# SymbolicML/DynamicExpressions.jl

Measured on AMD Instinct MI355X. Metric: node-evals/sec, higher is better.
Workload: dtype f32

## Files before the change

### dynamicexpressions.jl_amd/api.py

```python
from __future__ import annotations

import ctypes as C
import math
import os
from dataclasses import dataclass
from typing import Optional, Sequence, Tuple, Union

import numpy as np

from .node import Node, TAPE_DTYPE, count_constant_nodes, flatten_graph, flatten_population, max_feature, preserve_sharing
from .operators import OperatorEnum

_HERE = os.path.dirname(os.path.abspath(__file__))
LIB_PATH = os.environ.get("DE_HIP_LIB") or os.path.join(_HERE, "csrc", "libde_hip.so")

DE_F32, DE_F64, DE_F16, DE_CF32, DE_CF64 = 0, 1, 2, 3, 4
COMPLEX_DTYPES = (np.dtype(np.complex64), np.dtype(np.complex128))
GRAD_VARIABLE, GRAD_CONSTANT, GRAD_BOTH = 0, 1, 2
ABI_VERSION = 3
OPT_EARLY_EXIT, OPT_FUSE_DEG1, OPT_FUSE_DEG2, OPT_BUMPER_CHECKS, OPT_TURBO, OPT_FULL_EVAL, OPT_FORWARD_GRAD, OPT_REVERSE_GRAD = 1, 2, 4, 8, 16, 32, 64, 128

EXPORTS = [
    "de_abi_version", "de_opcode_table_version", "de_opcode_by_name", "de_opcode_name",
    "de_opcode_degree", "de_status_string", "de_ctx_create", "de_ctx_destroy", "de_ctx_set_stream",
    "de_ctx_synchronize", "de_ctx_declare_dataset", "de_ctx_stream", "de_last_error", "de_program_create", "de_program_create_cse",
    "de_program_set_consts", "de_program_update", "de_program_destroy", "de_program_n_trees", "de_program_n_nodes",
    "de_program_n_grad", "de_program_dump", "de_program_verify", "de_program_stream_hash", "de_host_pool_selftest", "de_lower_tape", "de_lower_tape_stage", "de_lower_tape_complex", "de_lower_tape_stage_complex", "de_lower_tape_grad", "de_eval", "de_eval_grad", "de_eval_diff", "de_eval_loss", "de_eval_loss_grad", "de_eval_loss_grad_by_class",
    "de_loss_spec_check", "de_eval_loss_ex", "de_eval_fit_stats", "de_eval_loss_gn", "de_gn_max_rows", "de_eval_loss_grad_ex", "de_eval_loss_grad_by_class_ex",
    "de_eval_pullback_dX", "de_eval_tree_array", "de_eval_plan", "de_prio_tiles_wanted", "de_program_last_live_trees", "de_dist_unique_id", "de_dist_init", "de_dist_destroy", "de_dist_shard_size", "de_dist_world_size",
    "de_dist_broadcast", "de_dist_gather_flags", "de_dist_last_error", "de_ctx_last_kernel_ms", "de_ctx_last_kernel_name",
    "de_ctx_device", "de_ctx_timing_ring", "de_ctx_timing_read", "de_dist_reorder_selftest", "de_eval_sum_certificate",
    "de_dist_set_timeout", "de_ctx_trim", "de_program_set_consts_device", "de_program_get_consts", "de_program_consts_device_path",
    "de_lower_tape_assured", "de_lower_tape_assured_parts", "de_gn_lm_step", "de_fit_consts_lm", "de_lm_solve_host",
    "de_gn_spec_check", "de_eval_loss_gn_ex", "de_fit_consts_lm_ex", "de_eval_fit_stats_grad",
    "de_gn_wide_max_rows", "de_eval_loss_gn_wide", "de_lm_solve_host_wide", "de_gn_lm_step_wide", "de_fit_consts_lm_wide",
    "de_lm_project_host", "de_fit_stats_lm_step", "de_fit_consts_lm_scaled",
    "de_eval_fit_stats_grad_wide", "de_lm_project_host_wide", "de_fit_stats_lm_step_wide", "de_fit_consts_lm_scaled_wide",
    "de_bfgs_max_rows", "de_bfgs_direction_host", "de_bfgs_update_host", "de_fit_consts_bfgs",
    "de_tape_params_to_consts", "de_eval_tree_params", "de_eval_loss_tree_params", "de_eval_loss_grad_tree_params",
    "de_tree_params_accumulate_host",
    "de_fit_tree_params_bfgs", "de_tree_params_pack_host", "de_tree_params_unpack_host",
]


class DeviceError(RuntimeError):
    """The HIP library/GPU is unavailable or a de_* call failed.  Never swallowed."""


class UncertifiedFlag(DeviceError):
    """EvalContext(strict_flags=True): the device's element-wise validity flag of this tree is not PROVABLY the reference's
    `isfinite(sum(x))` flag (a finite array whose sum may overflow): the caller keeps the CPU path for it."""


class ParamArgs(C.Structure):
    _fields_ = [("params", C.c_void_p), ("ld_params", C.c_int64), ("n_classes", C.c_int64),
                ("classes", C.c_void_p), ("classes_is_i64", C.c_int32), ("class_base", C.c_int32)]


class LossSpec(C.Structure):
    _fields_ = [("kind", C.c_int32), ("reserved", C.c_int32), ("param", C.c_double)]


class LmOpts(C.Structure):
    _fields_ = [("iters", C.c_int32), ("reserved", C.c_int32), ("lam0", C.c_double), ("up", C.c_double), ("down", C.c_double),
                ("lam_min", C.c_double)]


class TreeParams(C.Structure):
    _fields_ = [("params", C.c_void_p), ("ld_params", C.c_int64), ("n_classes", C.c_int64), ("n_params", C.c_int32),
                ("reserved", C.c_int32), ("class_starts", C.c_void_p), ("slot_param", C.c_void_p)]


class BfgsOpts(C.Structure):
    _fields_ = [("iters", C.c_int32), ("reserved", C.c_int32), ("step0", C.c_double), ("shrink", C.c_double), ("c1", C.c_double),
                ("curv", C.c_double)]


LOSS_KINDS = {"L2": 0, "L1": 1, "pullback": 2, "huber": 16, "logcosh": 17, "l1_eps": 18, "l2_eps": 19, "quantile": 20, "lp": 21,
              "logit_dist": 22, "logit_margin": 23, "l1_hinge": 24}


def loss_spec(loss: str, loss_param: float = 0.0, with_gradient: bool = True) -> LossSpec:
    if loss == "pullback" and not with_gradient:
        raise KeyError(loss)
    spec = LossSpec(LOSS_KINDS[loss], 0, float(loss_param))
    if library().de_loss_spec_check(C.byref(spec), int(with_gradient)) != 0:
        raise ValueError(f"loss {loss!r}: parameter {loss_param!r} is not finite or outside the kind's range (include/de_hip.h de_loss_kind_t)")
    return spec


def gn_loss_spec(loss: str, loss_param: float = 0.0, e_floor: float = 1e-4) -> LossSpec:
    spec = LossSpec(LOSS_KINDS[loss], 0, float(loss_param))
    rc = library().de_gn_spec_check(C.byref(spec), float(e_floor))
    if rc == 7:
# ... 375 lines not shown
    if lib.de_abi_version() != ABI_VERSION:
        raise DeviceError(f"{LIB_PATH} has ABI version {lib.de_abi_version()}, this module was written for {ABI_VERSION}: rebuild (csrc/build.sh)")
    lib.de_opcode_table_version.restype = C.c_int
    lib.de_opcode_by_name.argtypes = [C.c_char_p, C.c_int]
    lib.de_opcode_name.restype = C.c_char_p
    lib.de_opcode_name.argtypes = [C.c_int]
    lib.de_opcode_degree.argtypes = [C.c_int]
    lib.de_status_string.restype = C.c_char_p
    lib.de_status_string.argtypes = [C.c_int]
    lib.de_ctx_create.argtypes = [C.c_int, vp, C.POINTER(vp)]
    lib.de_ctx_destroy.argtypes = [vp]
    lib.de_ctx_set_stream.argtypes = [vp, vp]
    lib.de_ctx_synchronize.argtypes = [vp]
    lib.de_ctx_declare_dataset.argtypes = [vp, C.c_int, vp, i64, i64, i32]
    lib.de_ctx_stream.restype = vp
    lib.de_ctx_stream.argtypes = [vp]
    lib.de_last_error.restype = C.c_char_p
    lib.de_last_error.argtypes = [vp]
    lib.de_program_create.argtypes = [vp, C.c_int, vp, vp, i64, vp, vp, i32, i32, u32, C.POINTER(vp)]
    lib.de_program_create_cse.argtypes = [vp, C.c_int, vp, vp, vp, vp, i64, vp, vp, i32, i32, u32, C.POINTER(vp)]
    lib.de_program_set_consts.argtypes = [vp, vp]
    lib.de_program_set_consts_device.argtypes = [vp, vp]
    lib.de_program_get_consts.argtypes = [vp, vp]
    lib.de_program_consts_device_path.argtypes = [vp]
    lib.de_program_update.argtypes = [vp, vp, i64, vp, vp, vp, vp, vp, vp]
    lib.de_program_destroy.argtypes = [vp]
    lib.de_program_n_trees.restype = i64
    lib.de_program_n_trees.argtypes = [vp]
    lib.de_program_n_nodes.restype = i64
    lib.de_program_n_nodes.argtypes = [vp]
    lib.de_program_n_grad.restype = i64
    lib.de_program_n_grad.argtypes = [vp, i64, C.c_int]
    lib.de_program_verify.argtypes = [vp]
    lib.de_host_pool_selftest.restype = C.c_int64
    lib.de_host_pool_selftest.argtypes = [C.c_int64, C.POINTER(C.c_int32)]
    lib.de_program_stream_hash.restype = C.c_uint64
    lib.de_program_stream_hash.argtypes = [vp]
    lib.de_program_dump.restype = i64
    lib.de_program_dump.argtypes = [vp, i64, vp, i64, C.c_int]
    lib.de_lower_tape.restype = i64
    lib.de_lower_tape.argtypes = [C.c_int, vp, i64, vp, i64, i32, i32, u32, vp, i64, vp]
    lib.de_lower_tape_stage.restype = i64
    lib.de_lower_tape_stage.argtypes = [C.c_int, vp, i64, vp, i64, i32, i32, u32, C.c_int, vp, i64]
    for fn in (lib.de_lower_tape_complex, lib.de_lower_tape_stage_complex):
        fn.restype = i64
    lib.de_lower_tape_complex.argtypes = lib.de_lower_tape.argtypes
    lib.de_lower_tape_stage_complex.argtypes = lib.de_lower_tape_stage.argtypes
    if hasattr(lib, "de_lower_tape_assured"):
        lib.de_lower_tape_assured.restype = i64
        lib.de_lower_tape_assured.argtypes = [vp, i64, vp, i64, i32, u32, C.c_double, vp, i64]
    if hasattr(lib, "de_lower_tape_assured_parts"):
        lib.de_lower_tape_assured_parts.restype = i64
        lib.de_lower_tape_assured_parts.argtypes = [vp, i64, vp, i64, i32, u32, C.c_double, u32, vp, i64]
    lib.de_lower_tape_grad.restype = i64
    lib.de_lower_tape_grad.argtypes = [C.c_int, vp, i64, vp, i64, i32, i32, u32, C.c_int, C.c_int, vp, i64, vp]
    lib.de_eval.argtypes = [vp, vp, vp, i64, i64, C.POINTER(ParamArgs), vp, i64, vp]
    lib.de_eval_loss.argtypes = [vp, vp, vp, i64, i64, C.POINTER(ParamArgs), vp, vp, C.c_int32, vp, vp]
    lib.de_eval_loss_grad.argtypes = [vp, vp, vp, i64, i64, C.POINTER(ParamArgs), C.c_int, vp, vp, C.c_int32, vp, vp, vp, vp]
    lib.de_eval_loss_grad_by_class.argtypes = [vp, vp, vp, i64, i64, C.POINTER(ParamArgs), C.c_int, vp, vp, C.c_int32, vp, vp, vp, vp, vp, vp]
    lib.de_loss_spec_check.argtypes = [C.POINTER(LossSpec), C.c_int]
    lib.de_eval_loss_ex.argtypes = [vp, vp, vp, i64, i64, C.POINTER(ParamArgs), vp, vp, C.POINTER(LossSpec), vp, vp]
    lib.de_eval_fit_stats.argtypes = [vp, vp, vp, i64, i64, C.POINTER(ParamArgs), vp, vp, vp, vp, vp]
    lib.de_eval_loss_gn.argtypes = [vp, vp, vp, i64, i64, C.POINTER(ParamArgs), C.c_int, vp, vp, vp, vp, vp, vp, vp, vp]
    lib.de_gn_max_rows.argtypes = []
    if hasattr(lib, "de_fit_consts_lm"):
        lib.de_gn_lm_step.argtypes = [vp, C.c_int, i64, vp, vp, vp, vp, vp, vp, vp, vp]
        lib.de_fit_consts_lm.argtypes = [vp, vp, vp, i64, i64, C.POINTER(ParamArgs), vp, vp, C.POINTER(LmOpts), vp, vp, vp, vp]
        lib.de_lm_solve_host.argtypes = [C.c_int, vp, vp, C.c_double, vp]
    if hasattr(lib, "de_gn_spec_check"):
        lib.de_gn_spec_check.argtypes = [C.POINTER(LossSpec), C.c_double]
        lib.de_eval_loss_gn_ex.argtypes = [vp, vp, vp, i64, i64, C.POINTER(ParamArgs), C.c_int, vp, vp, C.POINTER(LossSpec), C.c_double,
                                           vp, vp, vp, vp, vp, vp]
        lib.de_fit_consts_lm_ex.argtypes = [vp, vp, vp, i64, i64, C.POINTER(ParamArgs), vp, vp, C.POINTER(LossSpec), C.c_double,
                                            C.POINTER(LmOpts), vp, vp, vp, vp]
    if hasattr(lib, "de_eval_fit_stats_grad"):
        lib.de_eval_fit_stats_grad.argtypes = [vp, vp, vp, i64, i64, C.POINTER(ParamArgs), C.c_int, vp, vp, vp, vp, vp, vp, vp, vp, vp]
    if hasattr(lib, "de_eval_loss_gn_wide"):
        lib.de_gn_wide_max_rows.argtypes = []
        lib.de_eval_loss_gn_wide.argtypes = lib.de_eval_loss_gn_ex.argtypes
        lib.de_lm_solve_host_wide.argtypes = lib.de_lm_solve_host.argtypes
        lib.de_gn_lm_step_wide.argtypes = lib.de_gn_lm_step.argtypes
        lib.de_fit_consts_lm_wide.argtypes = lib.de_fit_consts_lm_ex.argtypes
    if hasattr(lib, "de_fit_consts_lm_scaled"):
        lib.de_lm_project_host.argtypes = [C.c_int, vp, vp, vp, vp, vp, vp, vp]
        lib.de_fit_stats_lm_step.argtypes = [vp, C.c_int, i64, vp, vp, vp, vp, vp, vp, vp, vp, vp, vp, vp]
        lib.de_fit_consts_lm_scaled.argtypes = [vp, vp, vp, i64, i64, C.POINTER(ParamArgs), vp, vp, C.POINTER(LmOpts), vp, vp, vp, vp, vp, vp]
    if hasattr(lib, "de_fit_consts_lm_scaled_wide"):
        lib.de_eval_fit_stats_grad_wide.argtypes = lib.de_eval_fit_stats_grad.argtypes
        lib.de_lm_project_host_wide.argtypes = lib.de_lm_project_host.argtypes
        lib.de_fit_stats_lm_step_wide.argtypes = lib.de_fit_stats_lm_step.argtypes
        lib.de_fit_consts_lm_scaled_wide.argtypes = lib.de_fit_consts_lm_scaled.argtypes
    if hasattr(lib, "de_fit_consts_bfgs"):
        lib.de_bfgs_max_rows.argtypes = []
        lib.de_bfgs_direction_host.argtypes = [C.c_int, vp, vp, vp, vp, C.c_double, vp, vp]
        lib.de_bfgs_update_host.argtypes = [C.c_int, vp, vp, vp, vp, C.c_double]
        lib.de_fit_consts_bfgs.argtypes = [vp, vp, vp, i64, i64, C.POINTER(ParamArgs), vp, vp, C.POINTER(LossSpec), C.POINTER(BfgsOpts),
                                           vp, vp, vp, vp]
    if hasattr(lib, "de_eval_tree_params"):
        lib.de_tape_params_to_consts.restype = i64
        lib.de_tape_params_to_consts.argtypes = [vp, i64, i32, vp, vp, i64]
        lib.de_eval_tree_params.argtypes = [vp, vp, vp, i64, i64, C.POINTER(TreeParams), vp, i64, vp]
        lib.de_eval_loss_tree_params.argtypes = [vp, vp, vp, i64, i64, C.POINTER(TreeParams), vp, vp, C.POINTER(LossSpec), vp, vp]
        lib.de_eval_loss_grad_tree_params.argtypes = [vp, vp, vp, i64, i64, C.POINTER(TreeParams), vp, vp, C.POINTER(LossSpec), vp, vp, vp, vp, vp]
        lib.de_tree_params_accumulate_host.argtypes = [C.c_int, i32, vp, i32, i64, vp, vp, vp, vp, vp, vp, vp, vp]
    if hasattr(lib, "de_fit_tree_params_bfgs"):
        lib.de_fit_tree_params_bfgs.argtypes = [vp, vp, vp, i64, i64, C.POINTER(TreeParams), vp, vp, C.POINTER(LossSpec), C.POINTER(BfgsOpts),
# ... 195 lines not shown
        if not (X.stride(0) == 1 and (N <= 1 or X.stride(1) >= F)) and X.numel() > 0:
            X = X.t().contiguous().t()
        ld = X.stride(1) if N > 1 else max(F, 1)
        return X.data_ptr(), F, N, ld, X, True
    X = np.asarray(X)
    if X.ndim == 1:
        X = X.reshape(-1, 1)
    Xf = np.asfortranarray(X, dtype=dtype)
    F, N = Xf.shape
    return Xf.ctypes.data, F, N, max(F, 1), Xf, False


def lower_tape(tape, consts, n_features: int, n_params: int = 0, options: int = 7, dtype=np.float32):
    lib = library()
    dtype = np.dtype(dtype)
    tape = np.ascontiguousarray(tape)
    consts = np.ascontiguousarray(consts, dtype=dtype)
    meta = np.zeros(4, dtype=np.int32)
    cp = consts.ctypes.data if consts.size else None
    lower = lib.de_lower_tape_complex if dtype in COMPLEX_DTYPES else lib.de_lower_tape
    n = lower(_dtype_code(dtype), tape.ctypes.data, len(tape), cp, consts.size, n_features,
              n_params, options, None, 0, meta.ctypes.data)
    if n < 0:
        code = int(-n)
        name = lib.de_status_string(code).decode()
        if code == 3:
            from .operators import UnsupportedOperatorError
            raise UnsupportedOperatorError(name)
        raise ValueError(name)
    w = np.zeros(max(int(n), 1), dtype=np.uint32)
    lower(_dtype_code(dtype), tape.ctypes.data, len(tape), cp, consts.size, n_features,
          n_params, options, w.ctypes.data, w.size, meta.ctypes.data)
    return w[:int(n)].reshape(-1, 4), dict(n_slots=int(meta[0]), host_ok_eval=bool(meta[1]),
                                           host_ok_grad=bool(meta[2]), uses_params=bool(meta[3]))


def lower_tape_stage(tape, consts, n_features: int, stage: int, n_params: int = 0, options: int = 7,
                     dtype=np.float32) -> np.ndarray:
    lib = library()
    dtype = np.dtype(dtype)
    tape = np.ascontiguousarray(tape)
    consts = np.ascontiguousarray(consts, dtype=dtype)
    cp = consts.ctypes.data if consts.size else None
    args = (_dtype_code(dtype), tape.ctypes.data, len(tape), cp, consts.size, n_features, n_params, options, stage)
    stage_fn = lib.de_lower_tape_stage_complex if dtype in COMPLEX_DTYPES else lib.de_lower_tape_stage
    n = stage_fn(*args, None, 0)
    if n < 0:
        raise ValueError(lib.de_status_string(int(-n)).decode())
    w = np.zeros(max(int(n), 1), dtype=np.uint32)
    stage_fn(*args, w.ctypes.data, w.size)
    return w[:int(n)].reshape(-1, 4)


def lower_tape_assured(tape, consts, n_features: int, xmax: float = 64.0, options: int = 7, parts: Optional[int] = None) -> np.ndarray:
    lib = library()
    tape = np.ascontiguousarray(tape)
    consts = np.ascontiguousarray(consts, dtype=np.float32)
    cp = consts.ctypes.data if consts.size else None
    args = (tape.ctypes.data, len(tape), cp, consts.size, n_features, options, float(xmax))
    fn = lib.de_lower_tape_assured
    if parts is not None:
        fn, args = lib.de_lower_tape_assured_parts, args + (int(parts),)
    n = fn(*args, None, 0)
    if n < 0:
        raise ValueError(lib.de_status_string(int(-n)).decode())
    w = np.zeros(max(int(n), 1), dtype=np.float64)
    fn(*args, w.ctypes.data, w.size)
    return w[:int(n)].reshape(-1, 6)


def lower_tape_grad(tape, consts, n_features: int, mode: int, form: int, n_params: int = 0, options: int = 7, dtype=np.float32):
    lib = library()
    dtype = np.dtype(dtype)
    tape = np.ascontiguousarray(tape)
    consts = np.ascontiguousarray(consts, dtype=dtype)
    cp = consts.ctypes.data if consts.size else None
    meta = np.zeros(8, dtype=np.int32)
    args = (_dtype_code(dtype), tape.ctypes.data, len(tape), cp, consts.size, n_features, n_params, options, mode, form)
    n = lib.de_lower_tape_grad(*args, None, 0, meta.ctypes.data)
    if n < 0:
        raise ValueError(lib.de_status_string(int(-n)).decode())
    w = np.zeros(max(int(n), 1), dtype=np.uint32)
    lib.de_lower_tape_grad(*args, w.ctypes.data, w.size, meta.ctypes.data)
    return w[:int(n)].reshape(-1, 4), meta


def check_update_ids(indices, n_new: int, n_trees: int) -> np.ndarray:
    ids = np.asarray(list(indices) if not isinstance(indices, np.ndarray) else indices)
    if ids.ndim != 1:
        raise ValueError("update: indices must be one-dimensional")
    if len(ids) != n_new:
        raise ValueError(f"update: {len(ids)} indices for {n_new} trees")
    if len(ids) == 0:
        return np.zeros(0, dtype=np.int64)
    if ids.dtype.kind not in "iu":
        raise ValueError(f"update: indices must be integers, got {ids.dtype}")
    ids = np.ascontiguousarray(ids, dtype=np.int64)
    if ids.min() < 0 or ids.max() >= n_trees:
        raise ValueError(f"update: tree index outside [0, {n_trees})")
    if len(np.unique(ids)) != len(ids):
        raise ValueError("update: a tree index appears twice")
    return ids


class Population:

    def __init__(self, trees: Sequence[Node], operators: OperatorEnum, dtype=np.float32,
                 n_features: Optional[int] = None, n_params: int = 0,
                 eval_context: Optional[EvalContext] = None, ctx: Optional[Context] = None):
        self.ctx = ctx or default_context()
        self.dtype = np.dtype(dtype)
        self.operators = operators
        self.eval_context = eval_context or EvalContext()
        self.n_trees = len(trees)
# ... 138 lines not shown
        return library().de_program_consts_device_path(self._h) == 1

    def verify(self) -> None:
        self.ctx.check(library().de_program_verify(self._h))

    def stream_hash(self) -> int:
        return int(library().de_program_stream_hash(self._h))

    def _combine_rows(self, t: int, g, mode: int):
        if self._occ is None or self._occ[t] is None or mode == GRAD_VARIABLE:
            return g
        o = self._occ[t]
        lead = g.shape[0] - len(o)
        nu = int(o.max()) + 1
        if _is_torch(g):
            import torch
            out = torch.zeros((lead + nu,) + tuple(g.shape[1:]), dtype=g.dtype, device=g.device)
            out[:lead] = g[:lead]
            out.index_add_(0, torch.as_tensor(o + lead, device=g.device), g[lead:])
            return out
        out = np.zeros((lead + nu,) + g.shape[1:], dtype=g.dtype)
        out[:lead] = g[:lead]
        np.add.at(out, o + lead, g[lead:])
        return out

    def plan(self, N: int) -> dict:
        pl = np.zeros(3, dtype=np.int32)
        self.ctx.check(library().de_eval_plan(self._h, N, pl.ctypes.data))
        return dict(tile=int(pl[0]), n_chunks=int(pl[1]), trees_per_chunk=int(pl[2]))

    def last_live_trees(self) -> int:
        n = C.c_int64(-1)
        self.ctx.check(library().de_program_last_live_trees(self._h, C.byref(n)))
        return int(n.value)

    def n_grad(self, tree: int, mode: int) -> int:
        return int(library().de_program_n_grad(self._h, tree, mode))

    def _n_grad_all(self, mode: int) -> np.ndarray:
        cache = self.__dict__.setdefault("_ng_cache", {})
        if mode not in cache:
            lib = library()
            cache[mode] = np.array([lib.de_program_n_grad(self._h, t, mode) for t in range(self.n_trees)], dtype=np.int64)
        return cache[mode]

    def dump(self, tree: int) -> np.ndarray:
        lib = library()
        n = lib.de_program_dump(self._h, tree, None, 0, 0)
        w = np.zeros(max(int(n), 1), dtype=np.uint32)
        got = lib.de_program_dump(self._h, tree, w.ctypes.data, w.size, 0)
        return w[:int(got)].reshape(-1, 4)

    def meta(self, tree: int) -> dict:
        w = np.zeros(7, dtype=np.uint32)
        library().de_program_dump(self._h, tree, w.ctypes.data, 7, 1)
        return dict(n_slots=int(w[0]), host_ok_eval=bool(w[1]), host_ok_grad=bool(w[2]), uses_params=bool(w[3]), waves=int(w[4]),
                    assured=bool(w[5]), assured_valid=bool(w[6]))

    def dump_stage(self, tree: int, which: int) -> np.ndarray:
        lib = library()
        n = lib.de_program_dump(self._h, tree, None, 0, which)
        w = np.zeros(max(int(n), 1), dtype=np.uint32)
        got = lib.de_program_dump(self._h, tree, w.ctypes.data, w.size, which)
        return w[:int(got)].reshape(-1, 4)

    def _param_args(self, params, classes, class_base, N, keep):
        if self.n_params == 0 and params is None:
            return None
        if params is None or classes is None:
            raise ValueError("Incorrect call. You must pass the `classes::Vector` argument when calling `eval_tree_array`.")
        pa = ParamArgs()
        if _is_torch(params):
            import torch
            params = params.to(_torch_dtype(self.dtype))
            if params.stride(0) != 1 and params.numel() > 0:
                params = params.t().contiguous().t()
            P, ncls = params.shape
            pa.params, pa.ld_params = params.data_ptr(), (params.stride(1) if ncls > 1 else max(P, 1))
        else:
            params = np.asfortranarray(params, dtype=self.dtype)
            P, ncls = params.shape
            pa.params, pa.ld_params = params.ctypes.data, max(P, 1)
        if P != self.n_params:
            raise ValueError("parameter matrix has the wrong number of rows")
        if _is_torch(classes):
            import torch
            if classes.dtype not in (torch.int32, torch.int64):
                classes = classes.to(torch.int64)
            classes = classes.contiguous()
            n_c = classes.numel()
            key = (classes.data_ptr(), n_c, classes._version, ncls, class_base)
            if n_c and key not in self._classes_checked:
                mn, mx = int(classes.min().item()), int(classes.max().item())
                if mn < class_base or mx - class_base >= ncls:
                    raise ValueError(f"class ids must lie in [{class_base}, {class_base + ncls}): got [{mn}, {mx}] "
                                     "(maximum(classes) <= size(parameters, 2))")
                if len(self._classes_checked) > 64:
                    self._classes_checked.clear()
                self._classes_checked.add(key)
            pa.classes, pa.classes_is_i64 = classes.data_ptr(), int(classes.dtype == torch.int64)
        else:
            classes = np.ascontiguousarray(classes)
            if classes.dtype not in (np.int32, np.int64):
                classes = classes.astype(np.int64)
            n_c = classes.size
            if n_c:
                mn, mx = int(classes.min()), int(classes.max())
                if mn < class_base or mx - class_base >= ncls:
                    raise ValueError(f"class ids must lie in [{class_base}, {class_base + ncls}): got [{mn}, {mx}] "
                                     "(maximum(classes) <= size(parameters, 2))")
# ... 1367 lines not shown
```

### dynamicexpressions.jl_amd/csrc/de_api_eval.cpp

```cpp
#include "de_api_internal.h"

extern "C" {
int stage_in(de_ctx *c, DevBuf &buf, const void *user, size_t bytes, Staged *s) {
    s->dev = const_cast<void *>(user);
    s->staged = false;
    if (!user || bytes == 0 || is_device_ptr(user)) return DE_OK;
    HIP_TRY(c, buf.reserve(bytes));
    HIP_TRY(c, hipMemcpyAsync(buf.p, user, bytes, hipMemcpyHostToDevice, c->stream));
    s->dev = buf.p;
    s->staged = true;
    return DE_OK;
}
int stage_out(de_ctx *c, DevBuf &buf, void *user, size_t bytes, Staged *s) {
    s->dev = user;
    s->staged = false;
    if (!user || bytes == 0 || is_device_ptr(user)) return DE_OK;
    HIP_TRY(c, buf.reserve(bytes));
    s->dev = buf.p;
    s->staged = true;
    return DE_OK;
}

int check_param_args(de_ctx *c, const de_program *p, const de_param_args_t *pa, int64_t N) {
    if (!p->uses_params) return DE_OK;
// ... 236 lines not shown
    if (ok_dev) {
        sOk.dev = ok;
    } else {
        HIP_TRY(c, c->sOk.reserve((size_t)p->n_trees));
        sOk.dev = c->sOk.p;
        sOk.staged = true;
    }
    if (!p->d_ok_eval) HIP_TRY(c, hipMemcpyAsync(sOk.dev, p->host_ok_eval.data(), (size_t)p->n_trees, hipMemcpyHostToDevice, c->stream));
    if (p->uses_params) {
        rc = stage_in(c, c->sParams, pa->params, (size_t)pa->ld_params * (size_t)pa->n_classes * es, &sPar);
        if (rc) return rc;
        rc = stage_in(c, c->sClasses, pa->classes, (size_t)N * (pa->classes_is_i64 ? 8 : 4), &sCls);
        if (rc) return rc;
    }
    EvalArgs a;
    std::memset(&a, 0, sizeof a);
    a.code = p->d_code;
    a.code_off = p->d_code_off;
    a.n_trees = (int32_t)p->n_trees;
    a.n_slots = p->n_slots + (p->prows ? p->n_params : 0);
    a.prow_base = p->prows ? p->n_features + p->n_slots : 0;
    a.n_prows = p->prows ? p->n_params : 0;
    a.uses_params = p->uses_params;
    a.X = sX.dev;
    a.N = N;
    a.ldX = ldX;
    a.F = p->n_features;
    a.out = sOut.dev;
    a.ld_out = ld_out;
    a.ok = static_cast<uint8_t *>(sOk.dev);
    a.ok_init = p->d_ok_eval;
    if (p->uses_params) {
        a.params = sPar.dev;
        a.ld_params = pa->ld_params;
        a.n_classes = pa->n_classes;
        a.classes = sCls.dev;
        a.classes_is_i64 = pa->classes_is_i64;
        a.class_base = pa->class_base;
    }
    a.early_exit = (p->options & DE_OPT_EARLY_EXIT) != 0;
    a.skip_flagged = a.early_exit && !(p->options & DE_OPT_FULL_EVAL) && tree_skip_enabled();
    a.turbo = (p->options & DE_OPT_TURBO) != 0;
    a.threaded = p->threaded && !direct;
    a.direct = direct;
    a.loss = lr ? &la : nullptr;
    HIP_TRY(c, c->sPrio.reserve((size_t)3 * DE_PRIO_MAX_F * sizeof(unsigned long long)));
    a.prio_keys = c->sPrio.p;
    a.prio_keys_ready = !half && !cplx && !sX.staged && dataset_keys(c, p->dtype, X, N, ldX, p->n_features, &a.prio_keys);
    a.compact_code = p->d_compact_code;
    a.compact_ints = p->d_compact_ints;
    a.waves = p->waves;
    a.wave_slots = p->n_slots;
    a.var_stride = p->var_stride;
    a.assured = p->assured && p->assured_valid && p->var_stride != 0;
    a.assured_xmax = (float)p->assured_xmax;
    if (cr) {
        a.code = p->d_cert_code;
        a.code_off = p->d_cert_off;
        a.threaded = false;
        a.cert_max = c->sCert.p;
        a.out = nullptr;
        a.prio_keys = nullptr;
        a.compact_code = nullptr;
        a.compact_ints = nullptr;
    }
    if (!c->nested) HIP_TRY(c, time_begin(c));
    a.compacted = &p->last_compacted;
    p->last_compacted = false;
    if (half || cplx) {
        a.threaded = false;
        a.prio_keys = nullptr;
        a.compact_code = nullptr;
        a.compact_ints = nullptr;
    }
    if (half) HIP_TRY(c, launch_eval_f16(a, c->stream, &c->last_kernel));
    else if (cplx) HIP_TRY(c, launch_eval_complex(p->io, a, p->d_ctab, c->stream, &c->last_kernel));
    else HIP_TRY(c, launch_eval(p->dtype, a, c->stream, &c->last_kernel));
    if (!c->nested) HIP_TRY(c, time_end(c));
    if (sLoss.staged) HIP_TRY(c, hipMemcpyAsync(lr->loss, sLoss.dev, (size_t)p->n_trees * es, hipMemcpyDeviceToHost, c->stream));
    if (sStats.staged) HIP_TRY(c, hipMemcpyAsync(lr->stats, sStats.dev, (size_t)p->n_trees * 3 * sizeof(double), hipMemcpyDeviceToHost, c->stream));
    if (sYstats.staged) HIP_TRY(c, hipMemcpyAsync(lr->ystats, sYstats.dev, 3 * sizeof(double), hipMemcpyDeviceToHost, c->stream));
    if (sOut.staged) {
        if (ld_out == N)
            HIP_TRY(c, hipMemcpyAsync(out, sOut.dev, (size_t)p->n_trees * (size_t)N * es, hipMemcpyDeviceToHost, c->stream));
        else
            for (int64_t t = 0; t < p->n_trees; t++)
                HIP_TRY(c, hipMemcpyAsync(static_cast<char *>(out) + (size_t)t * (size_t)ld_out * es,
                                          static_cast<char *>(sOut.dev) + (size_t)t * (size_t)ld_out * es,
                                          (size_t)N * es, hipMemcpyDeviceToHost, c->stream));
    }
    if (sOk.staged) HIP_TRY(c, hipMemcpyAsync(ok, sOk.dev, (size_t)p->n_trees, hipMemcpyDeviceToHost, c->stream));
    if (cr) {
        std::vector<unsigned char> mx((size_t)p->n_trees * ces);
        std::vector<uint8_t> okh((size_t)p->n_trees);
        HIP_TRY(c, hipMemcpyAsync(mx.data(), c->sCert.p, mx.size(), hipMemcpyDeviceToHost, c->stream));
        HIP_TRY(c, hipMemcpyAsync(okh.data(), sOk.dev, okh.size(), hipMemcpyDeviceToHost, c->stream));
        HIP_TRY(c, hipStreamSynchronize(c->stream));
        const double top = half ? 65504.0 : p->dtype == DE_F32 ? (double)std::numeric_limits<float>::max() : std::numeric_limits<double>::max();
        double margin = 1.001;
        if (half) {
            const double d = 1024.0 + std::ceil(std::log2(std::max(1.0, (double)N / 1024.0))) + 8.0;
            margin = std::exp(d * std::log1p(std::ldexp(1.0, -11)));
        }
        for (int64_t t = 0; t < p->n_trees; t++) {
            double m = p->dtype == DE_F32 ? (double)reinterpret_cast<float *>(mx.data())[t] : reinterpret_cast<double *>(mx.data())[t];
            m = std::max(m, p->cert_cmax[(size_t)t]);
            if (cr->max_abs) cr->max_abs[t] = m;
            cr->certified[t] = (!okh[(size_t)t] || m * (double)N * margin < top || !(m == m)) ? 1 : 0;
// ... 41 lines not shown
```

### dynamicexpressions.jl_amd/csrc/de_api_internal.h

```cpp
#ifndef DE_API_INTERNAL_H
#define DE_API_INTERNAL_H
#include <hip/hip_runtime.h>
#include <pthread.h>

#include <chrono>
#include <cmath>
#include <cstdarg>
#include <cstdio>
#include <cstring>
#include <condition_variable>
#include <functional>
#include <map>
#include <mutex>
#include <memory>
#include <new>
#include <string>
#include <algorithm>
#include <array>
#include <atomic>
#include <thread>
#include <vector>

#include "../../include/de_hip.h"
#include "de_kernels.h"
// ... 71 lines not shown
    int dtype = DE_F32;
    int io = DE_F32;
    std::vector<double> consts_im, ctab;
    void *d_ctab = nullptr;
    uint32_t options = 0;
    int32_t n_features = 0, n_params = 0;
    int64_t n_trees = 0, n_nodes = 0;
    int n_slots = 0;
    bool prows = false;
    bool uses_params = false;
    std::vector<Instr> code;
    std::vector<int32_t> code_off;
    std::vector<int64_t> const_off;
    std::vector<int32_t> const_instr;
    std::vector<uint8_t> const_checks;
    std::vector<int32_t> n_consts_tree;
    bool cse_generic = false;
    std::vector<uint8_t> host_ok_eval;
    std::vector<uint8_t> host_ok_grad;
    std::vector<double> consts;
    bool folded = false;
    std::vector<Instr> fcode;
    std::vector<int32_t> fcode_off;
    std::vector<int32_t> fconst_instr;
    struct Fold { int32_t tree, instr; bool tested_always; };
    std::vector<Fold> folds;
    std::vector<int64_t> aux_const_src;
    de_program *aux = nullptr;
    std::vector<uint8_t> fold_ok;
    std::vector<uint8_t> fold_host;
    std::vector<int32_t> kfold;
    std::vector<int64_t> kf_csrc;
    char *d_kf = nullptr;
    size_t kf_o_noff = 0, kf_o_coff = 0, kf_o_cvals = 0, kf_o_out = 0, kf_o_ok = 0, kf_bytes = 0;
    std::vector<de_tape_node_t> fold_nodes;
    std::vector<int64_t> fold_noff, fold_coff;
    std::vector<int32_t> aux_fold;
    std::vector<int64_t> aux_csrc;
    std::vector<BoundInstr> bcode;
    std::vector<BoundInstr> tcode;
    std::vector<BoundInstr> fbcode;
    std::vector<int32_t> tcode_off;
    std::vector<BoundInstr> ccode;
    std::vector<int32_t> ccode_off;
    int waves = 1;
    int waves_choice = 0;
    int64_t var_stride = 0;
    std::vector<BoundInstr> ccode_w;
    bool assured = false, assured_valid = false;
    int assured_cfg = 0;
    double assured_xmax = 64.0;
    uint32_t assured_parts = 0;
    std::vector<uint32_t> aids;
    uint64_t end_handler = 0;
    uint64_t endv_handler[TOPX_ENDV_COUNT] = {0};
    bool threaded = false;
    bool direct = false;
    uint64_t handler_base = 0;
    std::vector<int32_t> bcode_off;
    BoundInstr *d_code = nullptr;
    int32_t *d_code_off = nullptr;
    bool eval_arena = false;
    BoundInstr *d_compact_code = nullptr;
    int32_t *d_compact_ints = nullptr;
    bool last_compacted = false;
    BoundInstr *d_cert_code = nullptr;
    int32_t *d_cert_off = nullptr;
    size_t cert_cap = 0;
    uint64_t consts_gen = 0;
    uint64_t cert_gen = ~0ull;
    std::vector<double> cert_cmax;
    BoundInstr *d_gcode = nullptr;
    int32_t *d_gcode_off = nullptr;
    std::vector<BoundInstr> gbcode;
    std::vector<int32_t> gbcode_off;
    bool gcode_stale = true;
    std::vector<BoundInstr> gtcode;
    std::vector<int32_t> gtcode_off;
    BoundInstr *d_gtcode = nullptr;
    int32_t *d_gtcode_off = nullptr;
    int32_t *d_gt_ids = nullptr;
    uint8_t *d_ok_eval = nullptr;
    uint8_t *d_ok_grad = nullptr;
    int32_t *d_ng = nullptr;
    int64_t *d_goff = nullptr;
    int tab_mode = -1;
    int64_t tab_N = -1;
    bool tab_ok_stale = true;
    std::vector<int32_t> bsite, tsite, gbsite, gtsite_of_gb;
    struct EvalSite { int32_t src, b, t, c; };
    struct GradSite { int32_t src, gb, gt, rt; };
    std::vector<EvalSite> eval_sites;
    std::vector<GradSite> grad_sites;
    uint64_t site_gen = 1, lists_gen = 0;
    std::vector<BoundInstr> rtcode;
    std::vector<int32_t> rtcode_off, rtcode_mid, rtsite_of_gb;
    BoundInstr *d_rtcode = nullptr;
    int32_t *d_rtcode_off = nullptr, *d_rtcode_mid = nullptr, *d_rt_ids = nullptr;
    int rt_mode = -1, rt_stage_cols = 0, rt_n_groups = 0;
    GradArgs::RevGroup rt_groups[8];
    bool rt_valid = false;
    uint64_t rt_handler_base = 0;
    uint32_t rt_param_off = 0;
    int gt_mode = -1;
    bool gt_valid = false, gt_wide = false;
    bool gt_share = false;
// ... 128 lines not shown
```

### dynamicexpressions.jl_amd/csrc/de_api_program.cpp

```cpp
#include "de_api_internal.h"
#include "de_const_patch.h"

template <typename T>
static bool host_fold_eval(const de_tape_node_t *nd, int64_t n, const double *consts, const int64_t *csrc, T *value, bool half = false) {
    T stack_small[32];
    std::vector<T> stack_big;
    T *st = stack_small;
    if (n > 32) { stack_big.resize((size_t)n); st = stack_big.data(); }
    int sp = 0;
    bool ok = true;
    for (int64_t i = 0; i < n; i++) {
        T v;
        if (nd[i].degree == 0) v = (T)consts[csrc[nd[i].arg]];
        else {
            const T b = st[--sp], a = st[--sp];
            switch (nd[i].op) {
            case DE_B_ADD: v = a + b; break;
            case DE_B_SUB: v = a - b; break;
            case DE_B_MUL: v = a * b; break;
            default: v = a / b; break;
            }
            if (half) v = (T)(_Float16)v;
        }
        ok = ok && std::isfinite(v);
// ... 81 lines not shown
    const std::vector<Instr> &src = p->folded ? p->fcode : p->code;
    const std::vector<int32_t> &off = p->folded ? p->fcode_off : p->code_off;
    const int nf = p->n_features;
    const de_program *old = ru && ru->old && same_binding(p, ru->old) ? ru->old : nullptr;
    build_stream_by_trees<BoundInstr>(p->n_trees, &p->bcode, &p->bcode_off, [&](int64_t t, std::vector<BoundInstr> *out) {
        if (old && ru->src[(size_t)t] >= 0) {
            const size_t s = (size_t)ru->src[(size_t)t];
            out->insert(out->end(), old->bcode.begin() + old->bcode_off[s], old->bcode.begin() + old->bcode_off[s + 1]);
            return;
        }
        const int32_t i0 = off[(size_t)t], i1 = off[(size_t)t + 1];
        bind_tree(src.data() + i0, (size_t)(i1 - i0), ee, nf, out, prb);
    });
    match_const_sites(src, off, p->bcode, p->bcode_off, p->n_trees, [](const BoundInstr &b) { return bop_is_const_source(b.bop); }, &p->bsite);
    p->tsite.clear();
    p->site_gen++;
}

static void make_chained(de_program *p);
static int choose_waves(const de_program *p) {
    if (TBLK != 64 || (p->uses_params && !p->prows)) return 1;
    if (const char *e = getenv("DE_EVAL_WAVES")) { const int v = atoi(e); return (v == 2 || v == 4 || v == 8) ? v : 1; }
    const size_t rb = trow_bytes(p->dtype), lds_cu = 160u << 10, shared = (size_t)p->n_features + (p->prows ? (size_t)p->n_params : 0);
    auto resident = [&](int W) -> size_t {
        const size_t lds = (shared + (size_t)W * (size_t)p->n_slots) * rb + (size_t)W * 256;
        const size_t by_regs = W >= 4 ? 7 / ((size_t)W / 4) : 28 / (size_t)W;
        return lds > 150u * 1024 ? 0 : std::min<size_t>(lds_cu / lds, by_regs) * (size_t)W;
    };
    int best = 1;
    size_t have = resident(1);
    for (int W : {2, 4, 8}) {
        const size_t w = resident(W);
        if (have >= 20) break;
        if (w * 2 < have * 3) {
            if (W == 2 && have < 12) continue;
            break;
        }
        best = W;
        have = w;
    }
    return best;
}
static void make_assured(de_program *p, const uint64_t *table);
static double assured_xmax_env() {
    const char *ax = getenv("DE_ASSURED_XMAX");
    const double xm = ax ? (double)(float)atof(ax) : 64.0;
    return (xm >= 0x1p-40 && xm <= 0x1p100) ? xm : 64.0;
}
static uint32_t assured_parts_env() {
    const char *ap = getenv("DE_ASSURED_PARTS");
    const int v = ap && *ap ? atoi(ap) : (int)ASSURED_PARTS_SHIPPED;
    return (uint32_t)v & ASSURED_PARTS_ALL;
}
static int make_threaded(de_ctx *c, de_program *p, const Reuse *ru = nullptr) {
    p->threaded = false;
    p->waves = 1;
    p->var_stride = 0;
    p->ccode_w.clear();
    p->assured = p->assured_valid = false;
    p->aids.clear();
    if (p->assured_cfg == 0) {
        if (ru && ru->old && ru->old->assured_cfg != 0) {
            p->assured_cfg = ru->old->assured_cfg;
            p->assured_xmax = ru->old->assured_xmax;
            p->assured_parts = ru->old->assured_parts;
        } else {
            const char *as = getenv("DE_ASSURED");
            p->assured_parts = assured_parts_env();
            p->assured_cfg = ((as && *as == '0') || p->assured_parts == 0) ? -1 : 1;
            p->assured_xmax = assured_xmax_env();
        }
    }
    dbg_lap(nullptr);
    p->direct = (size_t)eval_rows(p) * FLAT_ROW_BYTES > 150 * 1024;
    if (p->io == DE_F16) return DE_OK;
    if (is_complex_io(p->io)) {
        p->direct = (size_t)eval_rows(p) * complex_row_bytes(p->io) > 64 * 1024;
        return DE_OK;
    }
    if ((p->direct && ((size_t)eval_rows(p) + 3 * (size_t)p->n_slots) * trow_bytes(p->dtype) + 4 * 256 > 150 * 1024) || !eval_uses_threaded()) return DE_OK;
    if (eval_rows(p) > 4000) return DE_OK;
    uint64_t table[TOPX_TABLE];
    hipError_t st = eval_handler_table(p->dtype, (p->options & DE_OPT_TURBO) != 0, table);
    if (st != hipSuccess) return fail(c, DE_ERR_HIP, "handler table: %s", hipGetErrorString(st));
    dbg_lap("handler table");
    uint64_t base = table[0];
    for (int i = 0; i < (int)TOPX_TABLE; i++) base = std::min<uint64_t>(base, table[i]);
    for (int i = 0; i < (int)TOPX_TABLE; i++) {
        if (table[i] - base > 0xFFFFFFFFull) return DE_OK;
        if (p->dtype != DE_F32 && (table[i] >> 32) != (table[0] >> 32)) return DE_OK;
    }
    const bool hot_unary = !getenv("DE_NO_CONST_UNARY_HOT");
    const uint32_t row_bytes = (uint32_t)trow_bytes(p->dtype);
    const char *nf = getenv("DE_NO_FUSE");
    const bool fuse = !(nf && *nf == '1');
    if (p->waves_choice == 0) p->waves_choice = choose_waves(p);
    const int W = fuse ? p->waves_choice : 1;
    const int wave_prows = p->prows ? p->n_params : 0;
    const FuseRows rows0{(uint32_t)p->n_features, (uint32_t)(p->n_features + p->n_slots), 0, W > 1 ? wave_prows + (W - 1) * p->n_slots : 0};
    const de_program *old = ru && ru->old && ru->old->threaded && ru->old->waves_choice == p->waves_choice && same_binding(p, ru->old) ? ru->old : nullptr;
    build_stream_by_trees<BoundInstr>(p->n_trees, &p->fbcode, &p->tcode_off, [&](int64_t t, std::vector<BoundInstr> *out) {
        if (old && ru->src[(size_t)t] >= 0) {
            const size_t s = (size_t)ru->src[(size_t)t];
            out->insert(out->end(), old->fbcode.begin() + old->tcode_off[s], old->fbcode.begin() + old->tcode_off[s + 1]);
            return;
        }
        const int32_t b0 = p->bcode_off[(size_t)t], b1 = p->bcode_off[(size_t)t + 1];
        if (fuse) fuse_tree(p->bcode.data() + b0, (size_t)(b1 - b0), out, W > 1 && p->n_slots > 0 ? &rows0 : nullptr);
        else out->insert(out->end(), p->bcode.begin() + b0, p->bcode.begin() + b1);
    });
    dbg_lap("fuse_tree");
    p->tcode.resize(p->fbcode.size());
    auto threaded_words = [p, &table, base, hot_unary, row_bytes](const BoundInstr &b) {
        BoundInstr t = b;
        t.bop = (uint32_t)(table[b.bop] - base);
        if (hot_unary && (b.bop == BOP_GEN_ROW || b.bop == BOP_GEN_ACC)) {
            const int k = gun_index((int)(b.arg >> 24), DE_U_COS, DE_U_EXP, DE_U_SIN, DE_U_NEG, DE_U_SQUARE, DE_U_CUBE, DE_U_ABS, DE_U_LOG, DE_U_SAFE_LOG,
                                    DE_U_SQRT, DE_U_SAFE_SQRT, DE_U_TANH, DE_U_RELU);
            if (k >= 3) t.bop = (uint32_t)(table[TOPX_UN_BASE + (uint32_t)(k - 3) * 2 + (b.bop == BOP_GEN_ACC ? 1 : 0)] - base);
        }
        if (hot_unary && (b.bop == BOP_GEN_ROW || b.bop == BOP_GEN_CONST) && ((b.arg >> 24) == (uint32_t)DE_B_MAX || (b.arg >> 24) == (uint32_t)DE_B_MIN))
            t.bop = (uint32_t)(table[TOPX_BIN_BASE + ((b.arg >> 24) == (uint32_t)DE_B_MAX ? 0u : 2u) + (b.bop == BOP_GEN_CONST ? 1u : 0u)] - base);
        if (b.bop < BOP_COUNT && bop_is_const_source(b.bop)) {
// ... 100 lines not shown
        r.bop = la;
        if (f32) r.arg = lo;
        else { r.lo = lo; r.hi = hi; }
    };
    auto name_next = [&](BoundInstr &r, uint64_t handler) {
        if (f32) { r.lo = (uint32_t)handler; r.hi = (uint32_t)(handler >> 32); }
        else r.arg = (uint32_t)handler;
    };
    auto ev_of = [&](int64_t t) -> int {
        const int32_t i0 = p->tcode_off[(size_t)t], i1 = p->tcode_off[(size_t)t + 1];
        return i1 - i0 >= 2 ? topx_endv_of(p->fbcode[(size_t)i1 - 1].bop) : -1;
    };
    auto handler_of = [&](int32_t i, int32_t i1, int ev) -> uint64_t {
        return (i == i1 - 1 && ev >= 0) ? p->endv_handler[ev] : p->handler_base + p->tcode[(size_t)i].bop;
    };
    parallel_tree_ranges(p->n_trees, [&](int, int64_t tb, int64_t te) {
        for (int64_t t = tb; t < te; t++) {
            const int32_t i0 = p->tcode_off[(size_t)t], i1 = p->tcode_off[(size_t)t + 1];
            const size_t h = (size_t)i0 + (size_t)t + 1;
            p->ccode_off[(size_t)t] = (int32_t)h;
            const int ev = ev_of(t);
            for (int32_t i = i0; i < i1; i++) {
                const BoundInstr &s = p->tcode[(size_t)i];
                put(p->ccode[h + (size_t)(i - i0)], s.arg, s.lo, s.hi);
                if (i > i0) name_next(p->ccode[h + (size_t)(i - i0) - 1], handler_of(i, i1, ev));
            }
            put(p->ccode[h + (size_t)(i1 - i0)], (uint32_t)t, 0u, 0u);
            if (i1 > i0) name_next(p->ccode[h + (size_t)(i1 - i0) - 1], p->end_handler);
        }
    });
    for (int64_t t = 0; t < p->n_trees; t++) {
        const int32_t i0 = p->tcode_off[(size_t)t], i1 = p->tcode_off[(size_t)t + 1];
        const size_t h = (size_t)p->ccode_off[(size_t)t];
        const int ev = ev_of(t);
        if (i1 > i0) {
            const uint64_t first = handler_of(i0, i1, ev);
            name_next(p->ccode[h - 1], first);
            if (t > 0 && ev_of(t - 1) >= 0) name_next(p->ccode[h - 2], first);
        } else name_next(p->ccode[h - 1], p->end_handler);
        put(p->ccode[h - 1], t == 0 ? 0u : (uint32_t)(t - 1), (uint32_t)(i1 - i0) | (ev >= 0 ? DE_HDR_FUSED_END : 0u), 0u);
    }
    if (p->n_trees > 0) name_next(p->ccode.back(), p->end_handler);
    p->ccode_off[(size_t)p->n_trees] = (int32_t)p->ccode.size();
}
static inline void patch_chained_imm(de_program *p, int32_t c, uint32_t lo, uint32_t hi) {
    if (p->dtype == DE_F32) p->ccode[(size_t)c].arg = lo;
    else { p->ccode[(size_t)c].lo = lo; p->ccode[(size_t)c].hi = hi; }
    for (size_t w = 0; w * p->ccode.size() < p->ccode_w.size(); w++) {
        BoundInstr &r = p->ccode_w[w * p->ccode.size() + (size_t)c];
        if (p->dtype == DE_F32) r.arg = lo;
        else { r.lo = lo; r.hi = hi; }
    }
}
static void assured_link_trees(de_program *p, const uint64_t *table, int64_t tb, int64_t te, bool touched_only = false) {
    BoundInstr *cw = p->ccode_w.data();
    std::vector<AssuredInstr> info;
    auto name_next = [](BoundInstr &r, uint64_t handler) { r.lo = (uint32_t)handler; r.hi = (uint32_t)(handler >> 32); };
    auto ev_of = [&](int64_t t) -> int {
        const int32_t i0 = p->tcode_off[(size_t)t], i1 = p->tcode_off[(size_t)t + 1];
        return i1 - i0 >= 2 ? topx_endv_of(p->fbcode[(size_t)i1 - 1].bop) : -1;
    };
    for (int64_t t = tb; t < te; t++) {
        const int32_t i0 = p->tcode_off[(size_t)t], i1 = p->tcode_off[(size_t)t + 1];
        if (i1 <= i0) continue;
        if (touched_only && p->const_off[(size_t)t + 1] == p->const_off[(size_t)t]) continue;
        info.resize((size_t)(i1 - i0));
        assure_tree(p->fbcode.data() + i0, (size_t)(i1 - i0), p->n_features, p->assured_xmax, info.data(), p->assured_parts);
        const size_t h = (size_t)p->ccode_off[(size_t)t];
        const int ev = ev_of(t);
        for (int32_t i = i0; i < i1; i++) {
            const uint32_t id = info[(size_t)(i - i0)].id;
            p->aids[(size_t)i] = id;
            const uint64_t handler = (i == i1 - 1 && ev >= 0) ? (topx_enda_of(id) >= 0 && id != p->fbcode[(size_t)i].bop ? table[TOPX_ENDA_BASE + (uint32_t)topx_enda_of(id)] : p->endv_handler[ev])
                                     : id == p->fbcode[(size_t)i].bop ? p->handler_base + p->tcode[(size_t)i].bop : table[id];
            if (i > i0) name_next(cw[h + (size_t)(i - i0) - 1], handler);
            else {
                name_next(cw[h - 1], handler);
                if (t > 0 && ev_of(t - 1) >= 0) name_next(cw[h - 2], handler);
            }
        }
    }
}
static void make_assured(de_program *p, const uint64_t *table) {
    p->ccode_w = p->ccode;
    p->aids.assign(p->fbcode.size(), 0u);
    parallel_tree_ranges(p->n_trees, [&](int, int64_t tb, int64_t te) { assured_link_trees(p, table, tb, te); });
    p->var_stride = (int64_t)(p->bcode.size() + (size_t)p->n_trees + 2);
    p->assured = p->assured_valid = true;
}
static hipError_t upload_wave_variants(de_program *p) {
    for (size_t w = 0; p->var_stride && w * p->ccode.size() < p->ccode_w.size(); w++) {
        const hipError_t st = hipMemcpy(p->d_code + (w + 1) * (size_t)p->var_stride, p->ccode_w.data() + w * p->ccode.size(),
                                        p->ccode.size() * sizeof(BoundInstr), hipMemcpyHostToDevice);
        if (st != hipSuccess) return st;
    }
    return hipSuccess;
}

static void recompute_host_ok(de_program *p) {
    const bool ee = (p->options & DE_OPT_EARLY_EXIT) != 0;
    parallel_for_trees(p->n_trees, [&](int64_t t) {
        bool ok_eval = true, ok_grad = true;
        for (int64_t k = p->const_off[t]; k < p->const_off[t + 1]; k++) {
            const bool fin = finite_in(p->dtype, p->consts[k]) && (p->consts_im.empty() || finite_in(p->dtype, p->consts_im[k]));
            ok_grad = ok_grad && fin;
            const uint8_t ch = p->const_checks[k];
            if (!fin && ((ch & CONST_CHECK_ALWAYS) || (ee && (ch & CONST_CHECK_EE)))) ok_eval = false;
        }
        p->host_ok_eval[t] = ok_eval;
        p->host_ok_grad[t] = ok_grad;
    }, 1024);
    for (size_t j = 0; j < p->folds.size() && j < p->fold_ok.size(); j++)
        if (!p->fold_ok[j] && (p->folds[j].tested_always || ee)) p->host_ok_eval[(size_t)p->folds[j].tree] = 0;
}

static int create_impl(de_ctx_t *ctx, int dtype, const de_tape_node_t *nodes, const int64_t *node_offsets,
                       int64_t n_trees, const void *consts, const int64_t *const_offsets, int32_t n_features,
                       int32_t n_params, uint32_t options, bool allow_fold, de_program_t **out_program,
                       const de_tape_node_t *cse_nodes = nullptr, const int64_t *cse_offsets = nullptr, const Reuse *reuse = nullptr,
                       bool keep_input = true);

static int upload_ok_eval(de_ctx *c, de_program *p) {
    p->tab_ok_stale = true;
    if (p->n_trees == 0) return DE_OK;
    if (!p->d_ok_eval) HIP_TRY(c, hipMalloc(reinterpret_cast<void **>(&p->d_ok_eval), (size_t)std::max<int64_t>(p->n_trees, 1)));
    HIP_TRY(c, hipStreamSynchronize(c->stream));
    HIP_TRY(c, hipMemcpy(p->d_ok_eval, p->host_ok_eval.data(), (size_t)p->n_trees, hipMemcpyHostToDevice));
    return DE_OK;
}

static int refresh_folds(de_ctx *c, de_program *p, bool aux_current = false) {
    if (!p->folded || p->folds.empty()) return DE_OK;
    const size_t es = p->dtype == DE_F32 ? 4 : 8;
    const size_t ies = dtype_bytes(p->io);
    const size_t nf = p->folds.size();
    p->fold_ok.assign(nf, 0);
    parallel_for_trees((int64_t)nf, [&](int64_t j) {
        if (p->fold_host[(size_t)j] != 1) return;
        const de_tape_node_t *nd = p->fold_nodes.data() + p->fold_noff[(size_t)j];
// ... 564 lines not shown
                        std::vector<int32_t> oaux(o->folds.size(), -1);
                        for (size_t a = 0; a < o->aux_fold.size(); a++) oaux[(size_t)o->aux_fold[a]] = (int32_t)a;
                        aru.old = o->aux;
                        aru.src.assign(p->aux_fold.size(), -1);
                        for (size_t a = 0; a < p->aux_fold.size(); a++) {
                            const size_t j = (size_t)p->aux_fold[a];
                            const int64_t t = p->folds[j].tree;
                            if (!reuse->reuse(t)) continue;
                            const size_t s = (size_t)reuse->src[(size_t)t];
                            aru.src[a] = oaux[(size_t)(reuse->fold0[s] + ((int64_t)j - fold0[(size_t)t]))];
                        }
                        aru.fold0.assign((size_t)o->aux->n_trees + 1, 0);
                        for (const de_program::Fold &f : o->aux->folds) aru.fold0[(size_t)f.tree + 1]++;
                        for (size_t q = 0; q < (size_t)o->aux->n_trees; q++) aru.fold0[q + 1] += aru.fold0[q];
                    }
                    int rc = create_impl(ctx, io, xnodes.data(), xnoff.data(), (int64_t)p->aux_fold.size(), ac.data(),
                                         xcoff.data(), n_features, 0, options, false, &p->aux, nullptr, nullptr, aru.old ? &aru : nullptr,
                                         false);
                    if (rc != DE_OK) return rc;
                    lap("aux program (create)");
                }
                int rc = refresh_folds(ctx, p.get(), true);
                if (rc != DE_OK) return rc;
                lap("folds (evaluate: host + kernel + aux)");
            } else if (any_cse) {
                p->folded = true;
            } else {
                p->fcode.clear();
                p->fcode_off.clear();
            }
        }
        if (!allow_fold) parallel_for_trees(n_trees, [&](int64_t t) { Lowered done; std::swap(done, low[(size_t)t]); });
        lap("release lowerings");
        if (cplx) fill_ctab_consts(p.get());
        recompute_host_ok(p.get());
        rebind(p.get(), reuse);
        lap("bind");
    } catch (const std::bad_alloc &) {
        return fail(ctx, DE_ERR_HIP, "out of host memory");
    }
    HIP_TRY(ctx, hipSetDevice(ctx->device));
    {
        int rc = DE_OK;
        try { rc = make_threaded(ctx, p.get(), reuse); } catch (const std::bad_alloc &) { rc = fail(ctx, DE_ERR_HIP, "out of host memory"); }
        if (rc != DE_OK) return rc;
    }
    lap("threaded + chained records");
    if (cplx) {
        const int rc = upload_ctab(ctx, p.get());
        if (rc != DE_OK) return rc;
    }
    const size_t cbytes = (p->bcode.size() + (size_t)p->n_trees + 2) * sizeof(BoundInstr);
    {
        const size_t nvar = p->threaded && p->var_stride ? (p->assured ? 2 : (size_t)p->waves) : 1;
        if (nvar > 1 && (size_t)p->var_stride * sizeof(BoundInstr) != cbytes) return fail(ctx, DE_ERR_HIP, "wave-group stream variants: stride and arena disagree");
        const size_t abytes = p->threaded ? 2 * nvar * cbytes : cbytes;
        auto al = [](size_t x) { return (x + 255) & ~(size_t)255; };
        const size_t off_bytes = p->bcode_off.size() * sizeof(int32_t);
        const size_t ints_bytes = p->threaded ? ((size_t)2 * (size_t)p->n_trees + 5) * sizeof(int32_t) : 0;
        const size_t o_off = al(abytes), o_ints = o_off + al(off_bytes), o_ok = o_ints + al(ints_bytes);
        const size_t total = o_ok + al((size_t)std::max<int64_t>(p->n_trees, 1));
        const hipError_t ast = prog_malloc(ctx, reinterpret_cast<void **>(&p->d_code), total);
        if (ast != hipSuccess) return fail(ctx, DE_ERR_HIP, "hipMalloc failed: %s", hipGetErrorString(ast));
        if (!in_one_window(p->d_code, abytes)) return fail(ctx, DE_ERR_HIP, "instruction stream straddles a 4 GiB boundary");
        char *base = reinterpret_cast<char *>(p->d_code);
        p->eval_arena = true;
        p->d_code_off = reinterpret_cast<int32_t *>(base + o_off);
        p->d_ok_eval = reinterpret_cast<uint8_t *>(base + o_ok);
        if (p->threaded) {
            p->d_compact_code = p->d_code + nvar * cbytes / sizeof(BoundInstr);
            p->d_compact_ints = reinterpret_cast<int32_t *>(base + o_ints);
        }
        lap("hipMalloc (arena)");
        const std::vector<BoundInstr> &stream = p->threaded ? p->ccode : p->bcode;
        const std::vector<int32_t> &offs = p->threaded ? p->ccode_off : p->bcode_off;
        hipError_t st = hipSuccess;
        if (total <= (size_t)(128u << 10)) {
            std::vector<unsigned char> img(total, 0);
            if (!stream.empty()) std::memcpy(img.data(), stream.data(), stream.size() * sizeof(BoundInstr));
            for (size_t w = 1; w < nvar; w++)
                std::memcpy(img.data() + w * cbytes, p->ccode_w.data() + (w - 1) * p->ccode.size(), p->ccode.size() * sizeof(BoundInstr));
            std::memcpy(img.data() + o_off, offs.data(), off_bytes);
            if (p->n_trees > 0) std::memcpy(img.data() + o_ok, p->host_ok_eval.data(), (size_t)p->n_trees);
            st = hipMemcpy(base, img.data(), total, hipMemcpyHostToDevice);
        } else {
            st = hipMemset(p->d_code, 0, nvar * cbytes);
            if (st == hipSuccess && !stream.empty()) st = hipMemcpy(p->d_code, stream.data(), stream.size() * sizeof(BoundInstr), hipMemcpyHostToDevice);
            if (st == hipSuccess) st = upload_wave_variants(p.get());
            if (st == hipSuccess) st = hipMemcpy(p->d_code_off, offs.data(), off_bytes, hipMemcpyHostToDevice);
            if (st == hipSuccess && p->n_trees > 0) st = hipMemcpy(p->d_ok_eval, p->host_ok_eval.data(), (size_t)p->n_trees, hipMemcpyHostToDevice);
        }
        if (st != hipSuccess) {
            prog_free(ctx, p->d_code);
            p->d_code = nullptr;
            return fail(ctx, DE_ERR_HIP, "program upload failed: %s", hipGetErrorString(st));
        }
    }
    lap("memset + upload (stream, offsets, flags)");
    if (getenv("DE_VERIFY") && *getenv("DE_VERIFY") == '1') {
        const int rc = de_program_verify(p.get());
        if (rc != DE_OK) return rc;
    }
    *out_program = p.release();
    return DE_OK;
}

static void refresh_site_lists(de_program *p) {
// ... 66 lines not shown
    const auto t3 = now();
    if (cplx) return upload_ctab(ctx, p);
    const char *nopatch = getenv("DE_NO_CONST_PATCH");
    if (!(nopatch && *nopatch == '1') && p->threaded && !p->tsite.empty() && !p->bsite.empty()) {
        const std::vector<Instr> &src = p->folded ? p->fcode : p->code;
        const bool gpatch = p->d_gcode && !p->gcode_stale && !p->gbsite.empty();
        const bool tpatch = gpatch && p->gt_valid && !p->gtsite_of_gb.empty();
        const bool rpatch = gpatch && p->rt_valid && !p->rtsite_of_gb.empty();
        refresh_site_lists(p);
        try {
        parallel_tree_ranges((int64_t)p->eval_sites.size(), [&](int, int64_t sb, int64_t se) {
            for (size_t q = (size_t)sb; q < (size_t)se; q++) {
                const de_program::EvalSite &e = p->eval_sites[q];
                const uint32_t lo = src[(size_t)e.src].imm.u32[0], hi = src[(size_t)e.src].imm.u32[1];
                p->bcode[(size_t)e.b].lo = lo;
                p->bcode[(size_t)e.b].hi = hi;
                p->tcode[(size_t)e.t].lo = lo;
                p->tcode[(size_t)e.t].hi = hi;
                p->fbcode[(size_t)e.t].lo = lo;
                p->fbcode[(size_t)e.t].hi = hi;
                patch_chained_imm(p, e.c, lo, hi);
            }
        }, 4096);
        if (gpatch)
            parallel_tree_ranges((int64_t)p->grad_sites.size(), [&](int, int64_t sb, int64_t se) {
                for (size_t q = (size_t)sb; q < (size_t)se; q++) {
                    const de_program::GradSite &g = p->grad_sites[q];
                    const uint32_t lo = p->code[(size_t)g.src].imm.u32[0], hi = p->code[(size_t)g.src].imm.u32[1];
                    p->gbcode[(size_t)g.gb].lo = lo;
                    p->gbcode[(size_t)g.gb].hi = hi;
                    if (tpatch && g.gt >= 0) {
                        for (int64_t w = 0; w < (p->gt_share ? 4 : 1); w++) {
                            p->gtcode[(size_t)(g.gt + w * p->gt_stride)].lo = lo;
                            p->gtcode[(size_t)(g.gt + w * p->gt_stride)].hi = hi;
                        }
                    }
                    if (rpatch && g.rt >= 0) {
                        p->rtcode[(size_t)g.rt].lo = lo;
                        p->rtcode[(size_t)g.rt].hi = hi;
                    }
                }
            }, 4096);
        } catch (const std::bad_alloc &) { return fail(ctx, DE_ERR_HIP, "out of host memory"); }
        if (gpatch) {
            if (!tpatch) p->gt_valid = false;
            if (!rpatch) p->rt_valid = false;
        } else {
            p->gcode_stale = true;
        }
        if (p->assured) {
            uint64_t table[TOPX_TABLE];
            const hipError_t hs = eval_handler_table(p->dtype, (p->options & DE_OPT_TURBO) != 0, table);
            if (hs != hipSuccess) return fail(ctx, DE_ERR_HIP, "handler table: %s", hipGetErrorString(hs));
            parallel_tree_ranges(p->n_trees, [&](int, int64_t tb, int64_t te) { assured_link_trees(p, table, tb, te, true); });
            p->assured_valid = true;
        }
        const auto t4 = now();
        HIP_TRY(ctx, hipStreamSynchronize(ctx->stream));
        if (!p->ccode.empty())
            HIP_TRY(ctx, hipMemcpy(p->d_code, p->ccode.data(), p->ccode.size() * sizeof(BoundInstr), hipMemcpyHostToDevice));
        HIP_TRY(ctx, upload_wave_variants(p));
        if (gpatch) {
            if (!p->gbcode.empty())
                HIP_TRY(ctx, hipMemcpy(p->d_gcode, p->gbcode.data(), p->gbcode.size() * sizeof(BoundInstr), hipMemcpyHostToDevice));
            if (p->gt_valid && !p->gtcode.empty())
                HIP_TRY(ctx, hipMemcpy(p->d_gtcode, p->gtcode.data(), p->gtcode.size() * sizeof(BoundInstr), hipMemcpyHostToDevice));
            if (p->rt_valid && !p->rtcode.empty())
                HIP_TRY(ctx, hipMemcpy(p->d_rtcode, p->rtcode.data(), p->rtcode.size() * sizeof(BoundInstr), hipMemcpyHostToDevice));
        }
        if (timing)
            fprintf(stderr, "set_consts us: write %ld, refresh_folds %ld, flags %ld, patch %ld, upload %ld\n", us(t0, t1), us(t1, t2), us(t2, t3),
                    us(t3, t4), us(t4, now()));
        return DE_OK;
    }
    p->gcode_stale = true;
    try {
        rebind(p);
    } catch (const std::bad_alloc &) {
        return fail(ctx, DE_ERR_HIP, "out of host memory");
    }
    {
        int rc = DE_OK;
        try { rc = make_threaded(ctx, p); } catch (const std::bad_alloc &) { rc = fail(ctx, DE_ERR_HIP, "out of host memory"); }
        if (rc != DE_OK) return rc;
    }
    HIP_TRY(ctx, hipStreamSynchronize(ctx->stream));
    if (!p->bcode.empty())
        HIP_TRY(ctx, hipMemcpy(p->d_code, (p->threaded ? p->ccode : p->bcode).data(),
                               (p->threaded ? p->ccode : p->bcode).size() * sizeof(BoundInstr), hipMemcpyHostToDevice));
    if (p->threaded) HIP_TRY(ctx, upload_wave_variants(p));
    return DE_OK;
}

int consts_materialise(de_program *p) {
    if (!p || !p->consts_dev_ahead) return DE_OK;
    de_ctx *c = p->ctx;
    const size_t es = p->dtype == DE_F32 ? 4 : 8;
    try {
        std::vector<unsigned char> h(std::max<size_t>(p->consts.size(), 1) * es);
        HIP_TRY(c, hipSetDevice(c->device));
        HIP_TRY(c, hipMemcpyAsync(h.data(), p->d_cp_vals, p->consts.size() * es, hipMemcpyDeviceToHost, c->stream));
        HIP_TRY(c, hipStreamSynchronize(c->stream));
        p->consts_dev_ahead = false;
        const int rc = set_consts_nothrow(p, h.data());
        if (rc != DE_OK) p->consts_dev_ahead = true;
        return rc;
    } catch (const std::bad_alloc &) { return fail(c, DE_ERR_HIP, "out of host memory"); }
// ... 458 lines not shown
                                    (fb.bop >= TOPX_UN_BASE && fb.bop < TOPX_BIN_BASE && ((fb.bop - TOPX_UN_BASE) & 1)) ||
                                    (fb.bop >= TOPX_BIN_BASE && ((fb.bop - TOPX_BIN_BASE) & 1));
                if (!no_row) {
                    const uint64_t off = r.bop & 0xFFFFFFu;
                    if (off % trow_bytes(p->dtype) != 0 || off + trow_bytes(p->dtype) > lds_bytes) return bad("LDS operand offset outside the launch's allocation", t, i - i0, r.bop);
                    const bool pushes = (fb.bop >= TOP_LOADROW_BASE && fb.bop < TOP_LOADCONST_PUSH && ((fb.bop - TOP_LOADROW_BASE) & 2)) ||
                                        (fb.bop >= TOP_UNROW_BASE && fb.bop < TOP_BINROWC_BASE && ((fb.bop - TOP_UNROW_BASE) & 2)) ||
                                        (fb.bop >= TOP_BIN2_BASE && fb.bop < TOP_COUNT && ((fb.bop - TOP_BIN2_BASE) & 1));
                    if (pushes) {
                        const int64_t prow = (int64_t)(off / trow_bytes(p->dtype)) + (int8_t)(r.bop >> 24);
                        if (prow < p->n_features || prow >= spill_end) return bad("push row of a superinstruction outside the spill slots", t, i - i0, r.bop);
                    }
                    if (fb.bop >= TOP_BIN2_BASE && fb.bop < TOP_COUNT && !(((fb.bop - TOP_BIN2_BASE) >> 2) & 1)) {
                        const int64_t second = (int64_t)off + (int32_t)(f32 ? r.arg : r.lo);
                        if (second < 0 || second % (int64_t)trow_bytes(p->dtype) != 0 || (uint64_t)second + trow_bytes(p->dtype) > lds_bytes) return bad("second operand row of a two-operand form", t, i - i0, (uint64_t)second);
                    }
                }
                if (fb.bop == BOP_GEN_PARAM && (f32 ? r.arg : r.lo) != (uint32_t)rows * (uint32_t)trow_bytes(p->dtype)) return bad("class-row offset of a parameter operand", t, i - i0, r.arg);
            }
        }
        if (p->waves > 1 && p->ccode_w.size() != (p->var_stride ? p->ccode.size() * (size_t)(p->waves - 1) : 0)) return bad("stream variants of the wave group", -1, p->waves, p->ccode_w.size());
        const uint64_t rb = trow_bytes(p->dtype);
        for (size_t w = 1; p->var_stride && w < (size_t)p->waves; w++) {
            const BoundInstr *cw = p->ccode_w.data() + (w - 1) * p->ccode.size();
            const int64_t shift = (p->prows ? p->n_params : 0) + (int64_t)w * p->n_slots, rows_all = rows + (int64_t)(p->waves - 1) * p->n_slots;
            auto moved = [&](int64_t row0, int64_t roww) { return roww == (row0 >= p->n_features && row0 < spill_end ? row0 + shift : row0) && roww < rows_all; };
            for (int64_t t = 0; t < p->n_trees; t++) {
                const int32_t i0 = p->tcode_off[(size_t)t], i1 = p->tcode_off[(size_t)t + 1], h = p->ccode_off[(size_t)t];
                for (int32_t i = i0 - 1; i <= i1; i++) {
                    const BoundInstr &r0 = p->ccode[(size_t)(h + (i - i0))], &r = cw[(size_t)(h + (i - i0))];
                    const bool same_next = f32 ? (r.lo == r0.lo && r.hi == r0.hi) : r.arg == r0.arg;
                    if (!same_next) return bad("stream variant names another handler", t, i - i0, w);
                    if (i < i0 || i == i1) { if (std::memcmp(&r, &r0, sizeof r)) return bad("stream variant: header / end record differs", t, i - i0, w); continue; }
                    const BoundInstr &fb = p->fbcode[(size_t)i];
                    if (fb.bop == BOP_GEN_PARAM) { if (std::memcmp(&r, &r0, sizeof r)) return bad("stream variant: a gathered-parameter record differs", t, i - i0, w); continue; }
                    const uint64_t off0 = r0.bop & 0xFFFFFFu, off = r.bop & 0xFFFFFFu;
                    if (off0 % rb != 0 || off % rb != 0) { if (off != off0) return bad("stream variant: operand word", t, i - i0, r.bop); }
                    else if (!moved((int64_t)(off0 / rb), (int64_t)(off / rb))) return bad("stream variant: operand row", t, i - i0, r.bop);
                    const bool pushes = (fb.bop >= TOP_LOADROW_BASE && fb.bop < TOP_LOADCONST_PUSH && ((fb.bop - TOP_LOADROW_BASE) & 2)) ||
                                        (fb.bop >= TOP_UNROW_BASE && fb.bop < TOP_BINROWC_BASE && ((fb.bop - TOP_UNROW_BASE) & 2)) ||
                                        (fb.bop >= TOP_BIN2_BASE && fb.bop < TOP_COUNT && ((fb.bop - TOP_BIN2_BASE) & 1));
                    if (pushes ? !moved((int64_t)(off0 / rb) + (int8_t)(r0.bop >> 24), (int64_t)(off / rb) + (int8_t)(r.bop >> 24)) : (r.bop >> 24) != (r0.bop >> 24))
                        return bad("stream variant: push row / aux byte", t, i - i0, r.bop);
                    const bool row_row = fb.bop >= TOP_BIN2_BASE && fb.bop < TOP_COUNT && !(((fb.bop - TOP_BIN2_BASE) >> 2) & 1);
                    if (row_row || fb.bop == BOP_TERN) {
                        const int64_t s0 = (int64_t)off0 + (int32_t)(f32 ? r0.arg : r0.lo), s1 = (int64_t)off + (int32_t)(f32 ? r.arg : r.lo);
                        if (s1 < 0 || s1 % (int64_t)rb != 0 || !moved(s0 / (int64_t)rb, s1 / (int64_t)rb)) return bad("stream variant: second operand row", t, i - i0, (uint64_t)s1);
                    } else if (f32 ? r.arg != r0.arg : (r.lo != r0.lo || r.hi != r0.hi))
                        return bad("stream variant: immediate differs", t, i - i0, w);
                }
            }
        }
        if (p->assured) {
            if (p->waves != 1 || !f32 || p->ccode_w.size() != p->ccode.size() || p->aids.size() != p->fbcode.size() || (size_t)p->var_stride < p->ccode.size())
                return bad("assured stream layout", -1, p->waves, p->ccode_w.size());
            const BoundInstr *cw = p->ccode_w.data();
            std::vector<AssuredInstr> info;
            auto named = [](const BoundInstr &q) { return ((uint64_t)q.hi << 32) | q.lo; };
            for (size_t r = 0; r < p->ccode.size(); r++)
                if (cw[r].bop != p->ccode[r].bop || cw[r].arg != p->ccode[r].arg) return bad("assured stream: operand words differ", -1, (int64_t)r, cw[r].bop);
            for (int64_t t = 0; t < p->n_trees; t++) {
                const int32_t i0 = p->tcode_off[(size_t)t], i1 = p->tcode_off[(size_t)t + 1], h = p->ccode_off[(size_t)t];
                if (i1 <= i0) continue;
                info.resize((size_t)(i1 - i0));
                assure_tree(p->fbcode.data() + i0, (size_t)(i1 - i0), p->n_features, p->assured_xmax, info.data(), p->assured_parts);
                const int ev = i1 - i0 >= 2 ? topx_endv_of(p->fbcode[(size_t)i1 - 1].bop) : -1;
                for (int32_t i = i0; i < i1; i++) {
                    const uint32_t id = info[(size_t)(i - i0)].id;
                    if (p->assured_valid && id != p->aids[(size_t)i]) return bad("assured stream: stale twin id", t, i - i0, p->aids[(size_t)i]);
                    const uint32_t have = p->aids[(size_t)i];
                    if (have >= TOPX_COUNT) return bad("assured stream: handler id", t, i - i0, have);
                    const uint64_t want = (i == i1 - 1 && ev >= 0) ? (topx_enda_of(have) >= 0 && have != p->fbcode[(size_t)i].bop ? table[TOPX_ENDA_BASE + (uint32_t)topx_enda_of(have)] : p->endv_handler[ev])
                                          : (have == p->fbcode[(size_t)i].bop ? p->handler_base + p->tcode[(size_t)i].bop : table[have]);
                    if (named(cw[(size_t)(h + (i - i0) - 1)]) != want) return bad("assured stream: handler word", t, i - i0, named(cw[(size_t)(h + (i - i0) - 1)]));
                }
                if (ev < 0 && named(cw[(size_t)(h + (i1 - i0) - 1)]) != p->end_handler) return bad("assured stream: tree does not end in the end record", t, i1 - i0, 0);
                if (ev >= 0 && named(cw[(size_t)(h + (i1 - i0) - 1)]) != named(cw[(size_t)(h + (i1 - i0))])) return bad("assured stream: end-fused instruction and end record disagree", t, i1 - i0, 0);
            }
        }
    }
    return DE_OK;
}

int64_t de_program_dump(const de_program_t *p, int64_t tree, uint32_t *words, int64_t cap, int which) {
    if (!p || tree < 0 || tree >= p->n_trees) return -DE_ERR_INVALID_ARG;
    const bool assured_valid = p->assured && p->assured_valid;
    if (const int mrc = consts_materialise(const_cast<de_program_t *>(p))) return -mrc;
    if (which == 1) {
        if (cap < 4) return -DE_ERR_INVALID_ARG;
        words[0] = (uint32_t)p->n_slots;
        words[1] = p->host_ok_eval[(size_t)tree];
        words[2] = p->host_ok_grad[(size_t)tree];
        words[3] = p->uses_params;
        if (cap < 5) return 4;
        words[4] = (uint32_t)(p->threaded ? p->waves : 1);
        if (cap < 7) return 5;
        words[5] = p->threaded && p->assured ? 1u : 0u;
        words[6] = p->threaded && assured_valid ? 1u : 0u;
        return 7;
    }
    if (which == 4) {
        if (!p->threaded || !p->assured) return 0;
        const int32_t b0 = p->tcode_off[(size_t)tree], b1 = p->tcode_off[(size_t)tree + 1];
        const int64_t nb = (int64_t)(b1 - b0) * 4;
        if (!words || cap < nb) return nb;
        std::memcpy(words, p->fbcode.data() + b0, (size_t)nb * 4);
        for (int32_t i = b0; i < b1; i++) words[(size_t)(i - b0) * 4] = p->aids[(size_t)i];
        return nb;
    }
    if (which == 2) {
        const int32_t b0 = p->bcode_off[(size_t)tree], b1 = p->bcode_off[(size_t)tree + 1];
        const int64_t nb = (int64_t)(b1 - b0) * 4;
        if (!words || cap < nb) return nb;
        std::memcpy(words, p->bcode.data() + b0, (size_t)nb * 4);
        return nb;
    }
    if (which == 3) {
        if (!p->threaded) return 0;
        const int32_t b0 = p->tcode_off[(size_t)tree], b1 = p->tcode_off[(size_t)tree + 1];
        const int64_t nb = (int64_t)(b1 - b0) * 4;
        if (!words || cap < nb) return nb;
        std::memcpy(words, p->fbcode.data() + b0, (size_t)nb * 4);
        return nb;
    }
    const int32_t i0 = p->code_off[(size_t)tree], i1 = p->code_off[(size_t)tree + 1];
    const int64_t nw = (int64_t)(i1 - i0) * 4;
    if (!words || cap < nw) return nw;
    std::memcpy(words, p->code.data() + i0, (size_t)nw * 4);
    return nw;
}

static int64_t lower_tape_impl(int dtype, const de_tape_node_t *nodes, int64_t n_nodes, const void *consts, int64_t n_consts,
                               int32_t n_features, int32_t n_params, uint32_t options, uint32_t *words, int64_t cap, int32_t *meta);
static int64_t lower_tape_stage_impl(int dtype, const de_tape_node_t *nodes, int64_t n_nodes, const void *consts, int64_t n_consts,
                                     int32_t n_features, int32_t n_params, uint32_t options, int stage, uint32_t *words, int64_t cap);
int64_t de_lower_tape(int dtype, const de_tape_node_t *nodes, int64_t n_nodes, const void *consts,
                      int64_t n_consts, int32_t n_features, int32_t n_params, uint32_t options, uint32_t *words,
                      int64_t cap, int32_t *meta) {
    if (is_complex_io(dtype)) return -DE_ERR_INVALID_ARG;
    return lower_tape_impl(dtype, nodes, n_nodes, consts, n_consts, n_features, n_params, options, words, cap, meta);
}
int64_t de_lower_tape_complex(int dtype, const de_tape_node_t *nodes, int64_t n_nodes, const void *consts,
                              int64_t n_consts, int32_t n_features, int32_t n_params, uint32_t options, uint32_t *words,
                              int64_t cap, int32_t *meta) {
    if (!is_complex_io(dtype)) return -DE_ERR_INVALID_ARG;
    return lower_tape_impl(dtype, nodes, n_nodes, consts, n_consts, n_features, n_params, options, words, cap, meta);
}
int64_t de_lower_tape_stage(int dtype, const de_tape_node_t *nodes, int64_t n_nodes, const void *consts,
                            int64_t n_consts, int32_t n_features, int32_t n_params, uint32_t options, int stage,
                            uint32_t *words, int64_t cap) {
    if (is_complex_io(dtype)) return -DE_ERR_INVALID_ARG;
    return lower_tape_stage_impl(dtype, nodes, n_nodes, consts, n_consts, n_features, n_params, options, stage, words, cap);
}
int64_t de_lower_tape_stage_complex(int dtype, const de_tape_node_t *nodes, int64_t n_nodes, const void *consts,
                                    int64_t n_consts, int32_t n_features, int32_t n_params, uint32_t options, int stage,
                                    uint32_t *words, int64_t cap) {
    if (!is_complex_io(dtype)) return -DE_ERR_INVALID_ARG;
    return lower_tape_stage_impl(dtype, nodes, n_nodes, consts, n_consts, n_features, n_params, options, stage, words, cap);
}
static int64_t lower_tape_impl(int dtype, const de_tape_node_t *nodes, int64_t n_nodes, const void *consts, int64_t n_consts,
// ... 3 lines not shown
    const bool cplx = is_complex_io(io);
    if (dtype == DE_F16 || dtype == DE_CF32) dtype = DE_F32;
    else if (dtype == DE_CF64) dtype = DE_F64;
    if (cplx && complex_refused_op(nodes, n_nodes) >= 0) return -DE_ERR_UNSUPPORTED_OP;
    if (cplx && n_params > 0) return -DE_ERR_UNSUPPORTED;
    try {
        LowerOptions lo;
        lo.early_exit = (options & DE_OPT_EARLY_EXIT) != 0;
        lo.fuse1 = (options & DE_OPT_FUSE_DEG1) != 0;
        lo.fuse2 = (options & DE_OPT_FUSE_DEG2) != 0;
        lo.bumper = (options & DE_OPT_BUMPER_CHECKS) != 0;
        lo.n_features = n_features;
        lo.n_params = n_params;
        lo.dtype = dtype;
        for (int64_t i = 0; i < n_nodes; i++)
            if ((nodes[i].degree == 1 && nodes[i].op == DE_OP_SHARE) || (nodes[i].degree == 0 && nodes[i].op == DE_LEAF_SHARED)) lo.cse = true;
        TreeProgram tp;
        std::string why;
        int rc = lower_tree(nodes, n_nodes, n_consts, lo, &tp, &why);
        if (rc != DE_OK) return -rc;
        bool ok_eval = true, ok_grad = true;
        for (int64_t k = 0; k < n_consts; k++) {
            const double v = load_elem(io, consts, (size_t)k);
            if (tp.const_instr[(size_t)k] >= 0) {
                if (cplx) write_cidx(tp.code[(size_t)tp.const_instr[(size_t)k]], (size_t)k);
                else write_imm(tp.code[(size_t)tp.const_instr[(size_t)k]], dtype, v);
            }
            const bool fin = finite_in(dtype, v) && finite_in(dtype, load_elem_im(io, consts, (size_t)k));
            ok_grad = ok_grad && fin;
            const uint8_t ch = tp.const_checks[(size_t)k];
            if (!fin && ((ch & CONST_CHECK_ALWAYS) || (lo.early_exit && (ch & CONST_CHECK_EE)))) ok_eval = false;
        }
        if (meta) {
            meta[0] = tp.n_slots;
            meta[1] = ok_eval;
            meta[2] = ok_grad;
            meta[3] = tp.uses_params;
        }
        const int64_t nw = (int64_t)tp.code.size() * 4;
        if (!words || cap < nw) return nw;
        std::memcpy(words, tp.code.data(), (size_t)nw * 4);
        return nw;
    } catch (...) {
        return -DE_ERR_HIP;
    }
}

int64_t de_lower_tape_assured(const de_tape_node_t *nodes, int64_t n_nodes, const void *consts, int64_t n_consts, int32_t n_features,
                              uint32_t options, double xmax, double *out, int64_t cap) {
    return de_lower_tape_assured_parts(nodes, n_nodes, consts, n_consts, n_features, options, xmax, ASSURED_PARTS_CLASSIC, out, cap);
}
int64_t de_lower_tape_assured_parts(const de_tape_node_t *nodes, int64_t n_nodes, const void *consts, int64_t n_consts, int32_t n_features,
                                    uint32_t options, double xmax, uint32_t parts, double *out, int64_t cap) {
    if (parts & ~ASSURED_PARTS_ALL) return -DE_ERR_INVALID_ARG;
    if (!(xmax >= 0x1p-40 && xmax <= 0x1p100)) return -DE_ERR_INVALID_ARG;
    int64_t nw = lower_tape_stage_impl(DE_F32, nodes, n_nodes, consts, n_consts, n_features, 0, options, 3, nullptr, 0);
    if (nw < 0) return nw;
    try {
        std::vector<BoundInstr> f((size_t)nw / 4);
        nw = lower_tape_stage_impl(DE_F32, nodes, n_nodes, consts, n_consts, n_features, 0, options, 3, reinterpret_cast<uint32_t *>(f.data()), nw);
        if (nw < 0) return nw;
        const int64_t n = (int64_t)f.size() * 6;
        if (!out || cap < n) return n;
        std::vector<AssuredInstr> info(f.size());
        assure_tree(f.data(), f.size(), n_features, xmax, info.data(), parts);
        for (size_t i = 0; i < f.size(); i++) {
            double *o = out + 6 * i;
            o[0] = info[i].acc.lo; o[1] = info[i].acc.hi; o[2] = info[i].acc.amin; o[3] = info[i].acc.fin ? 1.0 : 0.0;
            o[4] = (double)info[i].id; o[5] = (double)info[i].bits;
        }
        return n;
    } catch (...) {
        return -DE_ERR_HIP;
    }
}

static int64_t lower_tape_stage_impl(int dtype, const de_tape_node_t *nodes, int64_t n_nodes, const void *consts, int64_t n_consts,
                                     int32_t n_features, int32_t n_params, uint32_t options, int stage, uint32_t *words, int64_t cap) {
    if (stage != 2 && stage != 3 && stage != 4) return -DE_ERR_INVALID_ARG;
    if (stage == 4 && dtype != DE_F32) return -DE_ERR_INVALID_ARG;
    std::vector<uint32_t> g;
    int64_t nw = lower_tape_impl(dtype, nodes, n_nodes, consts, n_consts, n_features, n_params, options, nullptr, 0, nullptr);
    if (nw < 0) return nw;
    try {
        g.resize((size_t)nw);
        nw = lower_tape_impl(dtype, nodes, n_nodes, consts, n_consts, n_features, n_params, options, g.data(), nw, nullptr);
        if (nw < 0) return nw;
        std::vector<BoundInstr> b, f;
        bind_tree(reinterpret_cast<const Instr *>(g.data()), (size_t)nw / 4, (options & DE_OPT_EARLY_EXIT) != 0, n_features, &b);
        if (stage >= 3 && dtype != DE_F16 && !is_complex_io(dtype)) fuse_tree(b.data(), b.size(), &f);
        if (stage == 4) {
            std::vector<AssuredInstr> info(f.size());
            assure_tree(f.data(), f.size(), n_features, assured_xmax_env(), info.data(), assured_parts_env());
            for (size_t i = 0; i < f.size(); i++) f[i].bop = info[i].id;
        }
        const std::vector<BoundInstr> &o = stage >= 3 ? f : b;
        const int64_t n = (int64_t)o.size() * 4;
        if (!words || cap < n) return n;
        std::memcpy(words, o.data(), (size_t)n * 4);
        return n;
    } catch (...) {
        return -DE_ERR_HIP;
    }
}

}
```

### dynamicexpressions.jl_amd/csrc/de_bind.cpp

```cpp
#include "de_bind.h"

#include <algorithm>
#include <cmath>
#include <cstring>
#include <limits>

#include "../../include/de_opcodes.h"

namespace de {
namespace {

int hot_binary_index(uint32_t op) {
    switch (op) {
    case DE_B_ADD: return 0;
    case DE_B_SUB: return 1;
    case DOP_RSUB: return 2;
    case DE_B_MUL: return 3;
    case DE_B_DIV: return 4;
    case DOP_RDIV: return 5;
    default: return -1;
    }
}
int hot_unary_index(uint32_t op) {
    switch (op) {
// ... 205 lines not shown
AssuredVal a_make(double lo, double hi, double amin) {
    const double W = 0x1p-20, T = 0x1p-140, BIG = 0x1p120;
    lo -= std::fabs(lo) * W + T;
    hi += std::fabs(hi) * W + T;
    if (!(lo >= -BIG && hi <= BIG && lo <= hi)) return a_unbounded();
    amin = amin * (1.0 - W) - T;
    if (!(amin > 0.0)) amin = 0.0;
    if (lo > 0.0) amin = std::max(amin, lo);
    if (hi < 0.0) amin = std::max(amin, -hi);
    return AssuredVal{lo, hi, amin, true};
}
AssuredVal a_const(uint32_t bits) {
    float c;
    std::memcpy(&c, &bits, 4);
    if (!std::isfinite(c)) return a_unbounded();
    return AssuredVal{(double)c, (double)c, std::fabs((double)c), true};
}
double a_absmax(const AssuredVal &a) { return std::max(std::fabs(a.lo), std::fabs(a.hi)); }
AssuredVal a_div(const AssuredVal &n, const AssuredVal &d) {
    if (!n.fin || !d.fin || !(d.amin > 0.0)) return a_unbounded();
    const double amin = n.amin / a_absmax(d);
    if (d.lo > 0.0 || d.hi < 0.0) {
        const double dl = std::max(d.amin, std::min(std::fabs(d.lo), std::fabs(d.hi))), dh = a_absmax(d), s = d.lo > 0.0 ? 1.0 : -1.0;
        const double q[4] = {s * n.lo / dl, s * n.lo / dh, s * n.hi / dl, s * n.hi / dh};
        return a_make(std::min(std::min(q[0], q[1]), std::min(q[2], q[3])), std::max(std::max(q[0], q[1]), std::max(q[2], q[3])), amin);
    }
    const double m = a_absmax(n) / d.amin;
    return a_make(-m, m, amin);
}
AssuredVal a_bin(int k, const AssuredVal &x, const AssuredVal &b) {
    if (!x.fin || !b.fin) return a_unbounded();
    switch (k) {
    case 0: return a_make(x.lo + b.lo, x.hi + b.hi, 0.0);
    case 1: return a_make(x.lo - b.hi, x.hi - b.lo, 0.0);
    case 2: return a_make(b.lo - x.hi, b.hi - x.lo, 0.0);
    case 3: {
        const double q[4] = {x.lo * b.lo, x.lo * b.hi, x.hi * b.lo, x.hi * b.hi};
        return a_make(std::min(std::min(q[0], q[1]), std::min(q[2], q[3])), std::max(std::max(q[0], q[1]), std::max(q[2], q[3])), x.amin * b.amin);
    }
    case 4: return a_div(x, b);
    case 5: return a_div(b, x);
    default: return a_unbounded();
    }
}
AssuredVal a_un(int k, const AssuredVal &x) {
    if (!x.fin) return a_unbounded();
    if (k == 0) return a_make(-1.0, 1.0, 0.0);
    if (k == 1) return a_make(std::exp(x.lo), std::exp(x.hi), 0.0);
    return a_unbounded();
}
}

void assure_tree(const BoundInstr *f, size_t n, int n_features, double xmax, AssuredInstr *out, uint32_t parts) {
    static thread_local std::vector<AssuredVal> slots;
    slots.clear();
    const AssuredVal feature{-xmax, xmax, (parts & ASSURED_PART_FUSED_DIV) ? 0x1p-39 : 0x1p-40, true};
    auto row_val = [&](uint32_t row) -> AssuredVal {
        if (row < (uint32_t)n_features) return feature;
        const size_t s = row - (uint32_t)n_features;
        return s < slots.size() ? slots[s] : a_unbounded();
    };
    auto push = [&](uint32_t row, const AssuredVal &v) {
        if (row < (uint32_t)n_features) return;
        const size_t s = row - (uint32_t)n_features;
        if (s >= slots.size()) slots.resize(s + 1, a_unbounded());
        slots[s] = v;
    };
    AssuredVal acc = a_unbounded();
    for (size_t i = 0; i < n; i++) {
        const BoundInstr &b = f[i];
        const uint32_t id = b.bop, row = b.arg & 0xFFFFFFu;
        const uint32_t prow = (uint32_t)((int32_t)row + (int32_t)(int8_t)(b.arg >> 24));
        uint32_t twin = id, bits = 0;
        AssuredVal un_arg = a_unbounded(), div_acc = a_unbounded(), div_row = a_unbounded();
        const bool validity = (parts & ASSURED_PART_VALIDITY) != 0;
        if (id == BOP_LOAD_ROW) acc = row_val(row);
        else if (id == BOP_LOAD_CONST) acc = a_const(b.lo);
        else if (id == BOP_PUSH) push(row, acc);
        else if (id == BOP_CHECK_ROW || id == BOP_CHECK_ACC) ;
        else if (id >= BOP_BIN_BASE && id < BOP_BIN_END) {
            const uint32_t v = id - BOP_BIN_BASE;
            div_acc = acc;
            div_row = (v & 2) ? a_const(b.lo) : row_val(row);
            acc = a_bin((int)(v >> 2), acc, div_row);
            if (validity && (v & 1) && acc.fin) { twin = id - 1; bits |= ASSURED_OUT; }
        } else if (id >= BOP_UN_BASE && id < BOP_UN_END) {
            const uint32_t v = id - BOP_UN_BASE;
            un_arg = (v & 2) ? row_val(row) : acc;
            acc = a_un((int)(v >> 2), un_arg);
            if (validity && (v & 1) && acc.fin) { twin = id - 1; bits |= ASSURED_OUT; }
        } else if (id >= TOP_LOADROW_BASE && id < TOP_LOADCONST_PUSH) {
            const uint32_t v = id - TOP_LOADROW_BASE;
            if (v & 2) push(prow, acc);
            acc = row_val(row);
            if (validity && (v & 1) && acc.fin) { twin = top_loadrow((v & 2) != 0, false); bits |= ASSURED_ROW; }
        } else if (id == TOP_LOADCONST_PUSH) {
            push(b.arg & 0xFFFFFFu, acc);
            acc = a_const(b.lo);
        } else if (id >= TOP_UNROW_BASE && id < TOP_BINROWC_BASE) {
            const uint32_t v = id - TOP_UNROW_BASE;
            bool chk = (v & 1) != 0, outc = ((v >> 2) & 1) != 0;
            const bool psh = ((v >> 1) & 1) != 0;
            if (psh) push(prow, acc);
            const AssuredVal x = row_val(row);
            un_arg = x;
            acc = a_un((int)(v >> 3), x);
            if (validity && chk && x.fin) { chk = false; bits |= ASSURED_ROW; }
            if (validity && outc && acc.fin) { outc = false; bits |= ASSURED_OUT; }
            twin = top_unrow((int)(v >> 3), outc, psh, chk);
// ... 61 lines not shown
```

### dynamicexpressions.jl_amd/csrc/de_bind.h

```cpp
#pragma once
#include <stdint.h>

#include <vector>

#include "de_program.h"

namespace de {

enum BoundOp : uint32_t {
    BOP_LOAD_ROW = 0,
    BOP_LOAD_CONST,
    BOP_PUSH,
    BOP_CHECK_ROW,
    BOP_CHECK_ACC,
    BOP_BIN_BASE,
    BOP_BIN_END = BOP_BIN_BASE + 24,
    BOP_UN_BASE = BOP_BIN_END,
    BOP_UN_END = BOP_UN_BASE + 12,
    BOP_GEN_ROW = BOP_UN_END,
    BOP_GEN_CONST,
    BOP_GEN_ACC,
    BOP_GEN_PARAM,
    BOP_TERN,
    BOP_INJ_ACC,
// ... 135 lines not shown

inline bool top_reads_acc(uint32_t top, int generic_degree) {
    if (top == BOP_LOAD_ROW || top == BOP_LOAD_CONST || top == BOP_CHECK_ROW || top == BOP_INJ_ROW) return false;
    if (top == BOP_GEN_ROW || top == BOP_GEN_CONST || top == BOP_GEN_PARAM) return generic_degree != 1 && generic_degree != 0;
    if (top >= BOP_UN_BASE && top < BOP_UN_END) return ((top - BOP_UN_BASE) & 2u) == 0;
    if (top < BOP_COUNT) return true;
    if (top >= TOP_LOADROW_BASE && top < TOP_LOADCONST_PUSH) return ((top - TOP_LOADROW_BASE) & 2u) != 0;
    if (top == TOP_LOADCONST_PUSH) return true;
    if (top >= TOP_UNROW_BASE && top < TOP_BINROWC_BASE) return ((top - TOP_UNROW_BASE) & 2u) != 0;
    if (top >= TOP_BINROWC_BASE && top < TOP_BIN2_BASE) return true;
    if (top >= TOP_BIN2_BASE && top < TOP_COUNT) return ((top - TOP_BIN2_BASE) & 1u) != 0;
    if (top >= TOPX_UN_BASE && top < TOPX_BIN_BASE) return ((top - TOPX_UN_BASE) & 1u) != 0;
    return true;
}

inline bool bop_reads_row(uint32_t bop) {
    if (bop == BOP_LOAD_ROW || bop == BOP_GEN_ROW) return true;
    if (bop >= BOP_BIN_BASE && bop < BOP_BIN_END) return ((bop - BOP_BIN_BASE) & 2u) == 0;
    return bop >= BOP_UN_BASE && bop < BOP_UN_END && ((bop - BOP_UN_BASE) & 2u) != 0;
}

inline bool top_carries_const(uint32_t top) {
    if (top < BOP_COUNT) return bop_is_const_source(top);
    if (top == TOP_LOADCONST_PUSH) return true;
    if (top >= TOP_BIN2_BASE && top < TOP_COUNT) return (((top - TOP_BIN2_BASE) >> 2) & 1u) != 0;
    return false;
}

struct FuseRows { uint32_t slot_lo, slot_hi; int32_t shift, headroom; };
void fuse_tree(const BoundInstr *b, size_t n, std::vector<BoundInstr> *out, const FuseRows *rows = nullptr);
bool top_is_const_source(uint32_t top);

struct AssuredVal {
    double lo, hi;
    double amin;
    bool fin;
};
enum : uint32_t { ASSURED_OUT = 1u,
                  ASSURED_ROW = 2u,
                  ASSURED_PRE = 4u,
                  ASSURED_DIV_ACC = 8u,
                  ASSURED_DIV_ROW = 16u,
                  ASSURED_DIV_A = 32u,
                  ASSURED_DIV_B = 64u };
constexpr uint32_t ASSURED_PARTS_SHIPPED = 31u;
enum : uint32_t { ASSURED_PART_VALIDITY = 1u, ASSURED_PART_PRETEST = 2u, ASSURED_PART_DIVISION = 4u, ASSURED_PART_FUSED_DIV = 8u, ASSURED_PART_END = 16u,
                  ASSURED_PARTS_CLASSIC = 7u, ASSURED_PARTS_ALL = 31u };
struct AssuredInstr {
    AssuredVal acc;
    uint32_t id;
    uint32_t bits;
};
void assure_tree(const BoundInstr *f, size_t n, int n_features, double xmax, AssuredInstr *out, uint32_t parts);

void bind_tree(const Instr *code, size_t n, bool early_exit, int n_features, std::vector<BoundInstr> *out, int param_row_base = -1, int slot_shift = 0);

}
```

### dynamicexpressions.jl_amd/csrc/de_kernels.h

```cpp
#pragma once
#include <hip/hip_runtime.h>
#include <stdint.h>

#include "../../include/de_hip.h"
#include "de_bind.h"
#include "de_program.h"

namespace de {

constexpr int BLOCK = 256;
#ifndef DE_TBLK
#define DE_TBLK 64
#endif
constexpr int TBLK = DE_TBLK, TWAVES = DE_TBLK / 64;
#ifndef DE_TG
#define DE_TG 1
#endif
constexpr int TG_F32 = DE_TG, TG_F64 = 1;
constexpr int tg_planes(int dtype) { return dtype == DE_F32 ? TG_F32 : TG_F64; }
constexpr int ttile_samples(int dtype) { return TBLK * tg_planes(dtype) * (dtype == DE_F32 ? 4 : 2); }
constexpr size_t trow_bytes(int dtype) { return (size_t)(TBLK * tg_planes(dtype) + 1) * 16; }
constexpr int flat_tile_samples(int io) { return io == DE_F32 || io == DE_F16 ? 1024 : (io == DE_CF64 ? 256 : 512); }
constexpr size_t FLAT_ROW_BYTES = 257 * 16;

struct LossArgs {
    const void *y;
    const void *w;
    int32_t kind;
    double param;
    double e_floor;
    void *partial;
    void *seg_sum;
    void *loss;
    double *stats;
    double *ystats;
};
constexpr int32_t FIT_STATS_KIND = 25;
constexpr int FIT_STATS_VALUES = 4;

struct EvalArgs {
    const BoundInstr *code;
    const int32_t *code_off;
    int32_t n_trees;
    int32_t n_slots;
    int32_t prow_base, n_prows;
    bool uses_params;
    const void *X;
    int64_t N, ldX;
    int32_t F;
    void *out;
    int64_t ld_out;
    uint8_t *ok;
    const uint8_t *ok_init;
    const void *params;
    int64_t ld_params;
    int64_t n_classes;
    const void *classes;
    int32_t classes_is_i64, class_base;
    bool early_exit;
    bool skip_flagged;
    bool turbo;
    bool threaded;
    bool direct;
    const LossArgs *loss;
    void *prio_keys;
    bool prio_keys_ready;
    void *compact_code;
    int32_t *compact_ints;
    bool *compacted;
    int32_t waves, wave_slots;
    int64_t var_stride;
    bool assured = false;
    float assured_xmax = 0.0f;
    void *cert_max;
};
constexpr int DE_PRIO_MAX_F = 8;
constexpr int DE_PRIO_UNIT = 64;
#define DE_FOLD_STACK 16
hipError_t launch_fold(int dtype, const void *nodes, const int64_t *noff, const int64_t *coff, const void *cvals, int64_t n_folds, void *out,
                       uint8_t *ok, hipStream_t stream);
hipError_t launch_dist_pack(uint8_t *send, const uint8_t *ok_local_dev, int64_t mine, int64_t per, hipStream_t stream);
hipError_t launch_dist_unpack(uint8_t *ok_global_dev, const uint8_t *recv, int64_t per, int32_t world, int64_t n_trees, hipStream_t stream);
hipError_t launch_tile_extremes(int dtype, const void *X, int64_t N, int64_t ldX, int F, void *keys, hipStream_t stream, const uint8_t *ok_init = nullptr,
                                uint8_t *ok = nullptr, int32_t n_ok = 0);
bool prio_tiles_wanted(int64_t N, int F, int64_t n_trees);

constexpr int DE_GN_MAX_ROWS = 8;
constexpr int FIT_COLS = 6;
constexpr int FIT_MODE_PLAIN = 1, FIT_MODE_JTJ = 2;
struct GradArgs {
    EvalArgs e;
    const BoundInstr *generic_code;
    int32_t mode;
    int32_t P;
    void *grad;
    const int64_t *grad_off;
    const int32_t *n_grad;
    int32_t max_grad;
    int32_t diff_direction;
    const LossArgs *loss;
    const int64_t *col_off;
    int64_t n_cols;
    void *dloss;
    const int64_t *dloss_off;
    bool gn;
    void *jtj;
    const int64_t *jtj_off;
    bool fit, fit_jtj;
    double *fit_seg;
    const BoundInstr *threaded_code;
    const BoundInstr *rev_code;
    const int32_t *rev_code_off, *rev_code_mid;
    const int32_t *rev_ids;
    int32_t rev_n_groups;
    const int64_t *rev_tile_range;
    int64_t rev_n_tiles;
    struct RevGroup { int32_t first, n, rows; } rev_groups[8];
    int32_t rev_stage_cols;
    uint64_t rev_handler_base;
    uint32_t rev_param_off;
    bool prio_ready;
    bool gt_share;
    int64_t gt_var_stride;
    int32_t n_buckets;
    struct Bucket {
        int32_t GC, VS;
// ... 58 lines not shown
```

### dynamicexpressions.jl_amd/csrc/de_kernels.hip

```cpp
#include <hip/hip_runtime.h>
#include <algorithm>
#include <map>
#include <mutex>
#include <type_traits>
#include <vector>

#include <cstdlib>
#include <cstring>

#include "de_bind.h"
#include "de_device_ops.h"
#include "de_kernels.h"
#include "de_loss_kinds.h"
#include "de_plan.h"
#include "de_real_vec.h"

namespace de {


template <typename T> struct KArgs {
    const BoundInstr *code;
    const int32_t *code_off;
    const T *X;
    T *out;
    uint8_t *ok;
    const T *params;
    const void *classes;
    int64_t N, ldX, ld_out, ld_params, n_tiles, n_classes;
    int32_t F, n_trees, trees_per_chunk, n_chunks, n_slots, xstride;
    int32_t prow_base, n_prows;
    const unsigned long long *prio;
    uint32_t n_prio_blocks, n_prio, prio_shift;
    int32_t classes_is_i64, class_base, vec_store;
    const T *y;
    const T *w;
    T *partial;
    int32_t loss_kind;
    uint32_t cls_row_off;
    int32_t x_vec;
    int32_t skip_flagged;
    uint32_t f_magic;
    const int32_t *live_idx;
    const int32_t *ctrl;
    int32_t map_group;
    void *cert_max;
    int32_t tail_split;
    int64_t var_stride;
    uint32_t list_off;
    T loss_param;
    const double *fit_ystats;
    int32_t assured;
    float assured_xmax;
};
__device__ __forceinline__ bool assured_value_ok(float v, float xmax) { return (__builtin_fabsf(v) <= xmax) & (__builtin_fabsf(v) >= 0x1p-39f); }
__device__ __forceinline__ bool assured_value_ok(double, float) { return false; }


__device__ __forceinline__ TileMap map_block_grouped(uint32_t bid, int32_t n_chunks, int64_t n_tiles, uint32_t grp) {
    TileMap m;
    const uint32_t xcd = bid & 7u, idx = bid >> 3;
    const uint32_t per = grp * (uint32_t)n_chunks;
    const uint32_t g = idx / per, r = idx - g * per;
    m.chunk = (int32_t)(r / grp);
    m.tile = ((int64_t)g * grp + (r - (uint32_t)m.chunk * grp)) * 8 + xcd;
    m.valid = m.tile < n_tiles;
    return m;
}

template <typename T>
__device__ __forceinline__ void stage_param_rows(const KArgs<T> &a, T *__restrict__ rows, int row_elems, int64_t base, int tile, int tid, int blk) {
    const int64_t last = a.N - 1;
    for (int j = tid; j < tile; j += blk) {
        int64_t jj = base + j;
        jj = jj < last ? jj : last;
        const int64_t cl = clamp_class((a.classes_is_i64 ? reinterpret_cast<const int64_t *>(a.classes)[jj]
                                                         : (int64_t) reinterpret_cast<const int32_t *>(a.classes)[jj]) - a.class_base, a.n_classes);
        const T *__restrict__ col = a.params + a.ld_params * cl;
        for (int p = 0; p < a.n_prows; p++) rows[(size_t)(a.prow_base + p) * row_elems + j] = col[p];
    }
}

template <typename T> struct PoisonOf { typedef T type; };
template <> struct PoisonOf<float> { typedef float type __attribute__((ext_vector_type(2))); };
template <typename T> struct TG { static constexpr int G = sizeof(T) == 4 ? DE_TG : 1; };
static_assert(DE_TG == TG_F32, "de_kernels.h TG_F32 and DE_TG disagree");
#define DE_PLANE_BYTES (DE_TBLK * 16u)
#if DE_TG == 1
#define FOR_PLANES if (constexpr int g = 0; true)
#else
#define FOR_PLANES DE_UNROLL for (int g = 0; g < TG<T>::G; g++)
#endif
template <typename T> struct __attribute__((packed, aligned(8))) HState {
    typename VecOf<T>::type acc[TG<T>::G];
    typename PoisonOf<T>::type poison;
};
template <typename T> struct __attribute__((packed, aligned(8))) BState {
    typename VecOf<T>::type acc;
    typename PoisonOf<T>::type poison;
};
template <typename T> struct HLoss { typename VecOf<T>::type v[2]; };
template <typename T> struct ImmBits;
template <> struct ImmBits<float> { typedef uint32_t type; };
template <> struct ImmBits<double> { typedef uint64_t type; };
template <typename T> __device__ __forceinline__ T imm_from(typename ImmBits<T>::type b);
template <> __device__ __forceinline__ float imm_from<float>(uint32_t b) { return __uint_as_float(b); }
template <> __device__ __forceinline__ double imm_from<double>(uint64_t b) { return __longlong_as_double((long long)b); }
#define HARGS BState<T> st, uint32_t la, typename ImmBits<T>::type imm
#define LDSP(T, addr) (reinterpret_cast<__attribute__((address_space(3))) typename VecOf<T>::type *>((uintptr_t)(addr)))
// ... 1124 lines not shown
__global__ void __launch_bounds__(DE_TBLK * WW) de_eval_threaded_kernel(const KArgs<T> a) {
    typedef typename VecOf<T>::type V;
    constexpr int VW = VecOf<T>::W;
    constexpr int BLK = DE_TBLK, G = TG<T>::G, PLANE = BLK * VW, TILE = PLANE * G, ROWV = BLK * G + 1;
    static_assert(WW == 1 || DE_TBLK == 64, "a wave group shares one 64-lane tile");
    constexpr int SBLK = BLK * WW;
    extern __shared__ __align__(16) unsigned char smem_base[];
    unsigned char *const smem_raw = smem_base + DE_SKIPLIST_BYTES;
    T *__restrict__ rows = reinterpret_cast<T *>(smem_raw);

    TileMap tm;
    int flag_protocol = a.skip_flagged;
    int32_t n_trees = a.n_trees, n_chunks = a.n_chunks, tpc = a.trees_per_chunk;
    if (a.ctrl) {
        const ConstI32Ptr ct = (ConstI32Ptr)(uintptr_t)a.ctrl;
        n_trees = ct[0];
        n_chunks = ct[1];
        tpc = ct[2];
        if (n_trees <= 0) return;
    }
    const int32_t host_groups = WW > 1 ? (a.n_chunks + WW - 1) / WW : a.n_chunks, groups = WW > 1 ? (n_chunks + WW - 1) / WW : n_chunks + a.tail_split - 1;
    if (blockIdx.x < a.n_prio_blocks) {
        const uint32_t k = blockIdx.x / (uint32_t)host_groups;
        if (k >= a.n_prio) return;
        tm.tile = (int64_t)((uint32_t)a.prio[k] >> a.prio_shift);
        tm.chunk = (int32_t)(blockIdx.x % (uint32_t)host_groups);
        tm.valid = tm.tile < a.n_tiles;
        flag_protocol = 1;
    } else tm = a.map_group > 0 ? map_block_grouped(blockIdx.x - a.n_prio_blocks, groups, a.n_tiles, (uint32_t)a.map_group)
                                : map_block(blockIdx.x - a.n_prio_blocks, groups, a.n_tiles);
    if (!tm.valid) return;
    const int stid = threadIdx.x;
    const int tid = WW > 1 ? (int)(threadIdx.x & 63u) : (int)threadIdx.x;
    const int wave = WW > 1 ? __builtin_amdgcn_readfirstlane((int)(threadIdx.x >> 6)) : 0;
    const int64_t base = tm.tile * TILE;
    const int64_t last = a.N - 1;
    if constexpr (WW > 1) tm.chunk = tm.chunk * WW + wave;
    int tA = tm.chunk * tpc;
    int tB = (tA + tpc < n_trees) ? tA + tpc : n_trees;
    if (WW > 1 && tm.chunk >= n_chunks) tA = tB = 0;
    if (WW == 1 && a.tail_split > 1 && tm.chunk >= n_chunks - 1) {
        const int b0 = (n_chunks - 1) * tpc, rem = n_trees - b0;
        const int sub = (rem + a.tail_split - 1) / a.tail_split;
        tA = b0 + (tm.chunk - (n_chunks - 1)) * sub;
        tB = tA + sub < n_trees ? tA + sub : n_trees;
        if (tA >= tB) return;
    }
    uint8_t f_first = 1;
    if (a.skip_flagged && (WW > 1 || tid < 64) && tA + tid < tB) f_first = skip_flag_load(a.ok + (a.live_idx ? a.live_idx[tA + tid] : tA + tid), flag_protocol, tm.tile);
    uint64_t *const mask_slot = reinterpret_cast<uint64_t *>(smem_raw + (size_t)BLK * G * 16);
    int32_t co_first = 0;
    if (a.skip_flagged && tA + (tid & 63) < tB) co_first = a.code_off[tA + (tid & 63)];
    constexpr bool ASSURABLE = WW == 1 && !PARAMS && sizeof(T) == 4 && DE_TBLK == 64;
    bool x_ok = true;
    {
        const uint32_t F = (uint32_t)a.F;
        const uint32_t total = (uint32_t)TILE * F;
        if (a.x_vec && base + TILE <= a.N) {
            const V *__restrict__ src = reinterpret_cast<const V *>(a.X + base * (int64_t)F);
            const uint32_t GF = (uint32_t)G * F;
            if constexpr (WW > 1) {
                const uint32_t nv = (uint32_t)BLK * GF;
                for (uint32_t i0 = 0; i0 * SBLK < nv; i0 += 8) {
                    V buf[8];
                    DE_UNROLL for (uint32_t u = 0; u < 8; u++)
                        if (stid + (i0 + u) * SBLK < nv) buf[u] = src[stid + (i0 + u) * SBLK];
                    DE_UNROLL for (uint32_t u = 0; u < 8; u++) {
                        if (stid + (i0 + u) * SBLK < nv) {
                            const uint32_t e = (stid + (i0 + u) * SBLK) * VW;
                            uint32_t j = a.f_magic ? __umulhi(e, a.f_magic) : e;
                            uint32_t f = e - j * F;
                            DE_UNROLL for (int c = 0; c < VW; c++) {
                                rows[f * (ROWV * VW) + j] = buf[u][c];
                                ++f;
                                if (f == F) { f = 0; ++j; }
                            }
                        }
                    }
                }
            } else
            for (uint32_t i0 = 0; i0 < GF; i0 += 8) {
                V buf[8];
                DE_UNROLL for (uint32_t u = 0; u < 8; u++)
                    if (i0 + u < GF) buf[u] = src[tid + (i0 + u) * BLK];
                DE_UNROLL for (uint32_t u = 0; u < 8; u++) {
                    if (i0 + u < GF) {
                        const uint32_t e = (tid + (i0 + u) * BLK) * VW;
                        uint32_t j = a.f_magic ? __umulhi(e, a.f_magic) : e;
                        uint32_t f = e - j * F;
                        DE_UNROLL for (int c = 0; c < VW; c++) {
                            if constexpr (ASSURABLE) x_ok &= assured_value_ok(buf[u][c], a.assured_xmax);
                            rows[f * (ROWV * VW) + j] = buf[u][c];
                            ++f;
                            if (f == F) { f = 0; ++j; }
                        }
                    }
                }
            }
        } else if (a.ldX == (int64_t)F && base + TILE <= a.N) {
            const T *__restrict__ src = a.X + base * (int64_t)F;
            for (uint32_t e = stid; e < total; e += SBLK) {
                const uint32_t j = e / F, f = e - j * F;
                const T v = src[e];
                if constexpr (ASSURABLE) x_ok &= assured_value_ok(v, a.assured_xmax);
                rows[f * (ROWV * VW) + j] = v;
            }
        } else {
            for (uint32_t e = stid; e < total; e += SBLK) {
                const uint32_t j = e / F, f = e - j * F;
                int64_t jj = base + j;
                jj = jj < last ? jj : last;
                const T v = a.X[f + a.ldX * jj];
                if constexpr (ASSURABLE) x_ok &= assured_value_ok(v, a.assured_xmax);
                rows[f * (ROWV * VW) + j] = v;
            }
        }
    }
    if (PARAMS && a.n_prows > 0) {
        stage_param_rows<T>(a, rows, ROWV * VW, base, TILE, stid, SBLK);
    } else if (PARAMS && WW == 1) {
        DE_UNROLL for (int g = 0; g < G; g++) {
            uint32_t cv[4] = {0u, 0u, 0u, 0u};
            DE_UNROLL for (int i = 0; i < VW; i++) {
                int64_t jj = base + g * PLANE + tid * VW + i;
                jj = jj < last ? jj : last;
                cv[i] = (uint32_t)((uint64_t)a.ld_params * sizeof(T) *
                                   (uint64_t)clamp_class((a.classes_is_i64 ? reinterpret_cast<const int64_t *>(a.classes)[jj]
                                                                           : (int64_t) reinterpret_cast<const int32_t *>(a.classes)[jj]) - a.class_base,
                                                         a.n_classes));
            }
            const uint64_t tab = (uint64_t)(uintptr_t)a.params;
            unsigned char *crow = smem_raw + a.cls_row_off + g * DE_PLANE_BYTES + tid * 16;
            if constexpr (sizeof(T) == 4) {
                *reinterpret_cast<U32x4 *>(crow) = U32x4{cv[0], cv[1], cv[2], cv[3]};
                *reinterpret_cast<U32x4 *>(crow + RowOf<T>::BYTES) = U32x4{(uint32_t)tab, (uint32_t)(tab >> 32), 0u, 0u};
            } else {
                *reinterpret_cast<U32x4 *>(crow) = U32x4{cv[0], cv[1], (uint32_t)tab, (uint32_t)(tab >> 32)};
            }
        }
    }
    if constexpr (LOSS) {
        if (a.loss_kind >= DE_LOSS_HUBER && stid == 0) *reinterpret_cast<T *>(smem_base + LossParamLds<T>::ADDR) = a.loss_param;
    }
    uint64_t m_first = 0ull;
    if constexpr (WW > 1) {
        if (a.skip_flagged) m_first = __ballot(f_first == 0);
    } else if (a.skip_flagged && tid < 64) {
        const uint64_t m0 = __ballot(f_first == 0);
        if (tid == 0) *mask_slot = m0;
    }
    __syncthreads();

    const bool assured_tile = ASSURABLE && a.assured != 0 && __ballot(!x_ok) == 0ull;
    const ConstU4Ptr code = (ConstU4Ptr)(uintptr_t)(a.code + (WW > 1 ? (int64_t)wave * a.var_stride : (assured_tile ? a.var_stride : (int64_t)0)));
    const uint32_t list_at = (WW > 1 && wave > 0) ? a.list_off + (uint32_t)(wave - 1) * DE_SKIPLIST_BYTES : 0u;
    const ConstI32Ptr code_off = (ConstI32Ptr)(uintptr_t)a.code_off;
    const bool full = base + TILE <= a.N;
    const uint32_t lds0 = (uint32_t)(uintptr_t)smem_raw + tid * 16;
    HLoss<T> yv, wv;
    DE_UNROLL for (int g = 0; g < 2; g++) { yv.v[g] = V{}; wv.v[g] = V{}; }
    if constexpr (LOSS) {
        DE_UNROLL for (int g = 0; g < G; g++) DE_UNROLL for (int i = 0; i < VW; i++) {
            const int64_t j = base + g * PLANE + tid * VW + i;
            const int64_t jj = j < last ? j : last;
            yv.v[g][i] = a.y[jj];
            wv.v[g][i] = j <= last ? (a.w ? a.w[jj] : T(1)) : T(0);
        }
        if (a.loss_kind == FIT_STATS_KIND) {
            const T ym = (T)a.fit_ystats[1];
            DE_UNROLL for (int g = 0; g < G; g++) DE_UNROLL for (int i = 0; i < VW; i++) yv.v[g][i] = yv.v[g][i] - ym;
        }
    }

    if (tA >= tB) return;
    const uint64_t ldo = (uint64_t)a.ld_out * sizeof(T);
    const int sub = 63;
    for (int t0 = tA; t0 < tB; t0 += sub) {
    const int t1 = t0 + sub < tB ? t0 + sub : tB;
    uint64_t skip = 0ull;
    if (a.skip_flagged) {
        if constexpr (WW > 1) {
            if (t0 != tA) break;
            skip = ((uint64_t)(uint32_t)__builtin_amdgcn_readfirstlane((int)(uint32_t)(m_first >> 32)) << 32) | (uint64_t)(uint32_t)__builtin_amdgcn_readfirstlane((int)(uint32_t)m_first);
            skip &= (1ull << (t1 - t0)) - 1ull;
        } else {
        if (t0 != tA) {
            __syncthreads();
            if (tid < 64) {
                const int i = t0 + tid;
                const uint8_t f = i >= t1 ? (uint8_t)1 : skip_flag_load(a.ok + (a.live_idx ? a.live_idx[i] : i), flag_protocol, tm.tile);
                const uint64_t m0 = __ballot(f == 0);
                if (tid == 0) *mask_slot = m0;
            }
            __syncthreads();
        }
        {
            const uint64_t m = *mask_slot;
            skip = ((uint64_t)(uint32_t)__builtin_amdgcn_readfirstlane((int)(uint32_t)(m >> 32)) << 32) | (uint64_t)(uint32_t)__builtin_amdgcn_readfirstlane((int)(uint32_t)m);
            skip &= (1ull << (t1 - t0)) - 1ull;
        }
        }
        {
            const int i = t0 + (tid & 63);
            if (i < t1 && !((skip >> (tid & 63)) & 1ull)) {
                const uint32_t r = (uint32_t)__builtin_popcountll((~skip & ((1ull << (t1 - t0)) - 1ull)) >> 1 >> (tid & 63));
                const uint64_t hdr = (uint64_t)(uintptr_t)(code + (t0 == tA ? co_first : a.code_off[i]) - 1);
                reinterpret_cast<uint32_t *>(smem_base + list_at)[r] = (uint32_t)hdr;
// ... 361 lines not shown
#define DE_TEV(FF) case FF: hipLaunchKernelGGL((de_tile_extremes_vec_kernel<FF>), gv, dim3(256), 0, stream, x, N, shift, k, ok_init, ok, n_ok); break;
            DE_TEV(1) DE_TEV(2) DE_TEV(3) DE_TEV(4) DE_TEV(5) DE_TEV(6) DE_TEV(7) DE_TEV(8)
#undef DE_TEV
            default: return hipErrorInvalidValue;
        }
        return hipGetLastError();
    }
    if (dtype == DE_F32)
        hipLaunchKernelGGL((de_tile_extremes_kernel<float, DE_PRIO_MAX_F>), grid, dim3(256), 0, stream, static_cast<const float *>(X), N, ldX, F, shift,
                           static_cast<unsigned long long *>(keys), ok_init, ok, n_ok);
    else
        hipLaunchKernelGGL((de_tile_extremes_kernel<double, DE_PRIO_MAX_F>), grid, dim3(256), 0, stream, static_cast<const double *>(X), N, ldX, F, shift,
                           static_cast<unsigned long long *>(keys), ok_init, ok, n_ok);
    return hipGetLastError();
}
bool prio_tiles_wanted(int64_t N, int F, int64_t n_trees) {
    return F >= 1 && F <= DE_PRIO_MAX_F && n_trees >= env_int("DE_PRIO_MIN_TREES", 96) && (N + 255) / 256 >= env_int("DE_PRIO_MIN_TILES", 512) &&
           !env_int("DE_NO_PRIO_TILES", 0);
}

template <typename T>
static hipError_t launch_threaded_t(const EvalArgs &e, hipStream_t stream, const char **kname) {
    constexpr int VW = VecOf<T>::W;
    constexpr int TILE = TBLK * VW * TG<T>::G;
    KArgs<T> a;
    a.code = e.code;
    a.code_off = e.code_off;
    a.X = static_cast<const T *>(e.X);
    a.out = static_cast<T *>(e.out);
    a.ok = e.ok;
    a.params = static_cast<const T *>(e.params);
    a.classes = e.classes;
    a.N = e.N;
    a.ldX = e.ldX;
    a.ld_out = e.ld_out;
    a.ld_params = e.ld_params;
    a.prow_base = e.prow_base;
    a.n_prows = e.n_prows;
    a.n_tiles = (e.N + TILE - 1) / TILE;
    a.F = e.F;
    a.n_trees = e.n_trees;
    a.n_slots = e.n_slots;
    a.xstride = 0;
    a.classes_is_i64 = e.classes_is_i64;
    a.class_base = e.class_base;
    a.n_classes = e.n_classes > 0 ? e.n_classes : 1;
    a.vec_store = (reinterpret_cast<uintptr_t>(e.out) % 16 == 0 && (e.ld_out * sizeof(T)) % 16 == 0 && (uint64_t)e.ld_out * sizeof(T) < (1ull << 32)) ? 1 : 0;
    a.x_vec = (e.F >= 1 && e.ldX == e.F && reinterpret_cast<uintptr_t>(e.X) % 16 == 0 && (int64_t)TILE * e.F < 0x10000000LL) ? 1 : 0;
    a.f_magic = e.F > 1 ? (uint32_t)((0x100000000ull + (uint64_t)e.F - 1) / (uint64_t)e.F) : 0u;
    if (!env_int("DE_X_VEC", 1)) { a.x_vec = 0; a.f_magic = 0; }
    if (env_int("DE_DEBUG_NO_STORE", 0)) a.vec_store = 2;
    const int WW = (TBLK == 64 && (e.waves == 2 || e.waves == 4 || e.waves == 8) && (!e.uses_params || e.n_prows > 0)) ? e.waves : 1;
    a.var_stride = WW > 1 ? e.var_stride : 0;
    a.assured = (WW == 1 && TBLK == 64 && sizeof(T) == 4 && e.assured && e.var_stride != 0 && !e.uses_params) ? 1 : 0;
    a.assured_xmax = e.assured_xmax;
    if (a.assured) a.var_stride = e.var_stride;
    const unsigned n_variants = a.var_stride ? (a.assured ? 2u : (unsigned)WW) : 1u;
    int32_t tpc, nch, nc0;
    plan_chunks(e.n_trees, a.n_tiles, &nch, &tpc, &nc0, WW);
    a.trees_per_chunk = tpc;
    a.n_chunks = nch;
    a.live_idx = a.ctrl = nullptr;
    a.cert_max = nullptr;
    a.skip_flagged = (e.early_exit && e.skip_flagged && a.F + a.n_slots >= 1) ? 1 : 0;
    if (a.skip_flagged) { const int pr = env_int("DE_SKIP_PROTOCOL", (e.loss && tpc >= 8) ? 1 : 2); a.skip_flagged = pr >= 1 && pr <= 3 ? pr : 2; }
    const int64_t tiles8 = (a.n_tiles + 7) / 8;
    a.map_group = 0;
    if (a.n_tiles >= 64 && a.n_chunks > 1) {
        const int64_t g = env_int("DE_MAP_GROUP", (int64_t)a.F * 8 <= (int64_t)a.trees_per_chunk * WW ? (int)(tiles8 > 0x3fffffff ? 0x3fffffff : tiles8) : 0);
        a.map_group = (int32_t)(g <= 0 ? 0 : (g > tiles8 ? tiles8 : g));
    }
    const int64_t tiles8g = a.map_group > 0 ? (tiles8 + a.map_group - 1) / a.map_group * a.map_group : tiles8;
    a.tail_split = 1;
    const int64_t fills = (a.n_tiles * (int64_t)a.n_chunks) / ((int64_t)(cu_count() > 0 ? cu_count() : 256) * 21);
    if (TBLK == 64 && WW == 1 && a.map_group > 0 && a.n_chunks > 1 && fills <= env_int("DE_TAIL_SPLIT_FILLS", 24)) {
        const int ts = env_int("DE_TAIL_SPLIT", 4);
        const int most = tpc / 8;
        a.tail_split = ts < 1 ? 1 : (ts > most ? (most < 1 ? 1 : most) : ts);
    }
    auto groups_of = [&](int64_t chunks) { return WW > 1 ? (chunks + WW - 1) / WW : chunks + a.tail_split - 1; };
    int64_t blocks = tiles8g * 8 * groups_of(a.n_chunks);
    if (blocks <= 0 || blocks > 0x7fffffffLL) return hipErrorInvalidValue;
    a.prio = nullptr;
    a.n_prio_blocks = a.n_prio = 0;
    bool ok_set = !e.ok_init;
    if (TBLK == 64 && a.skip_flagged && e.prio_keys && a.F >= 1 && prio_tiles_wanted(a.N, a.F, a.n_trees)) {
        const int np = 3 * a.F;
        hipError_t ps = e.prio_keys_ready ? hipSuccess
                                          : launch_tile_extremes(sizeof(T) == 4 ? DE_F32 : DE_F64, a.X, a.N, a.ldX, a.F, e.prio_keys, stream, e.ok_init, e.ok, e.n_trees);
        if (ps != hipSuccess) return ps;
        ok_set = !e.prio_keys_ready;
        const int tile_samples = TILE;
        a.prio_shift = 0;
        while ((DE_PRIO_UNIT << a.prio_shift) < tile_samples) ++a.prio_shift;
        a.prio = static_cast<const unsigned long long *>(e.prio_keys);
        a.n_prio = (uint32_t)np;
        a.n_prio_blocks = (uint32_t)(((int64_t)np * (WW > 1 ? groups_of(a.n_chunks) : (int64_t)a.n_chunks) + 7) / 8 * 8);
        if (!env_int("DE_PRIO_PROBE", 1)) {
            a.tail_split = 1;
            blocks = tiles8g * 8 * groups_of(a.n_chunks);
        }
        blocks += a.n_prio_blocks;
        if (blocks > 0x7fffffffLL) return hipErrorInvalidValue;
    }
    if (!ok_set) {
        const hipError_t cs = hipMemcpyAsync(e.ok, e.ok_init, (size_t)e.n_trees, hipMemcpyDeviceToDevice, stream);
        if (cs != hipSuccess) return cs;
    }
    a.cls_row_off = (uint32_t)((size_t)(a.F + a.n_slots) * RowOf<T>::BYTES);
    const int prm_rows = (e.uses_params && e.n_prows == 0) ? (sizeof(T) == 4 ? 2 : 1) : 0;
// ... 233 lines not shown
```

### include/de_hip.h

```cpp
#ifndef DE_HIP_H
#define DE_HIP_H

#include <stddef.h>
#include <stdint.h>

#include "de_opcodes.h"

#ifdef __cplusplus
extern "C" {
#endif

#define DE_HIP_ABI_VERSION 3

typedef enum de_status {
    DE_OK = 0,
    DE_ERR_INVALID_ARG = 1,
    DE_ERR_BAD_TAPE = 2,
    DE_ERR_UNSUPPORTED_OP = 3,
    DE_ERR_HIP = 4,
    DE_ERR_NO_DEVICE = 5,
    DE_ERR_OUT_OF_RANGE = 6,
    DE_ERR_UNSUPPORTED = 7,
    DE_ERR_RCCL = 8
} de_status_t;
// ... 35 lines not shown
const char *de_status_string(int status);

#define DE_STREAM_NULL ((void *)(intptr_t)-1)
int de_ctx_create(int device, void *stream, de_ctx_t **out_ctx);
int de_ctx_destroy(de_ctx_t *ctx);
int de_ctx_set_stream(de_ctx_t *ctx, void *stream);
int de_ctx_synchronize(de_ctx_t *ctx);
int de_ctx_trim(de_ctx_t *ctx);
int de_ctx_declare_dataset(de_ctx_t *ctx, int dtype, const void *X, int64_t N, int64_t ldX, int32_t n_features);
void *de_ctx_stream(de_ctx_t *ctx);
int de_ctx_device(de_ctx_t *ctx);
const char *de_last_error(de_ctx_t *ctx);

int de_program_create(de_ctx_t *ctx, int dtype, const de_tape_node_t *nodes,
                      const int64_t *node_offsets, int64_t n_trees, const void *consts,
                      const int64_t *const_offsets, int32_t n_features, int32_t n_params,
                      uint32_t options, de_program_t **out_program);
int de_program_create_cse(de_ctx_t *ctx, int dtype, const de_tape_node_t *nodes, const int64_t *node_offsets,
                          const de_tape_node_t *cse_nodes, const int64_t *cse_offsets, int64_t n_trees,
                          const void *consts, const int64_t *const_offsets, int32_t n_features,
                          int32_t n_params, uint32_t options, de_program_t **out_program);
int de_program_set_consts(de_program_t *prog, const void *consts);
int de_program_set_consts_device(de_program_t *prog, const void *d_consts);
int de_program_get_consts(de_program_t *prog, void *out);
int de_program_consts_device_path(const de_program_t *prog);
int de_program_update(de_program_t *prog, const int64_t *tree_ids, int64_t n_update,
                      const de_tape_node_t *nodes, const int64_t *node_offsets,
                      const de_tape_node_t *cse_nodes, const int64_t *cse_offsets,
                      const void *consts, const int64_t *const_offsets);
int de_program_destroy(de_program_t *prog);
int64_t de_program_n_trees(const de_program_t *prog);
int64_t de_program_n_nodes(const de_program_t *prog);
int64_t de_program_n_grad(const de_program_t *prog, int64_t tree, int mode);
int64_t de_program_dump(const de_program_t *prog, int64_t tree, uint32_t *words, int64_t cap,
                        int which);

int de_program_verify(const de_program_t *prog);

uint64_t de_program_stream_hash(const de_program_t *prog);

int64_t de_host_pool_selftest(int64_t n, int32_t *n_ranges);

int64_t de_lower_tape(int dtype, const de_tape_node_t *nodes, int64_t n_nodes, const void *consts,
                      int64_t n_consts, int32_t n_features, int32_t n_params, uint32_t options,
                      uint32_t *words, int64_t cap, int32_t *meta);
int64_t de_lower_tape_stage(int dtype, const de_tape_node_t *nodes, int64_t n_nodes,
                            const void *consts, int64_t n_consts, int32_t n_features,
                            int32_t n_params, uint32_t options, int stage, uint32_t *words,
                            int64_t cap);
int64_t de_lower_tape_assured(const de_tape_node_t *nodes, int64_t n_nodes, const void *consts, int64_t n_consts,
                              int32_t n_features, uint32_t options, double xmax, double *out, int64_t cap);
int64_t de_lower_tape_assured_parts(const de_tape_node_t *nodes, int64_t n_nodes, const void *consts, int64_t n_consts,
                                    int32_t n_features, uint32_t options, double xmax, uint32_t parts, double *out, int64_t cap);
int64_t de_lower_tape_complex(int dtype, const de_tape_node_t *nodes, int64_t n_nodes, const void *consts,
                              int64_t n_consts, int32_t n_features, int32_t n_params, uint32_t options,
                              uint32_t *words, int64_t cap, int32_t *meta);
int64_t de_lower_tape_stage_complex(int dtype, const de_tape_node_t *nodes, int64_t n_nodes,
                                    const void *consts, int64_t n_consts, int32_t n_features,
                                    int32_t n_params, uint32_t options, int stage, uint32_t *words,
                                    int64_t cap);
int64_t de_lower_tape_grad(int dtype, const de_tape_node_t *nodes, int64_t n_nodes, const void *consts, int64_t n_consts,
                           int32_t n_features, int32_t n_params, uint32_t options, int mode, int form, uint32_t *words,
                           int64_t cap, int32_t *meta);
int64_t de_tape_params_to_consts(const de_tape_node_t *nodes, int64_t n_nodes, int32_t n_params, de_tape_node_t *out_nodes,
                                 int32_t *slot_param, int64_t cap);

typedef struct de_param_args {
    const void *params;
    int64_t ld_params;
    int64_t n_classes;
    const void *classes;
    int32_t classes_is_i64;
    int32_t class_base;
} de_param_args_t;

int de_eval(de_ctx_t *ctx, de_program_t *prog, const void *X, int64_t N, int64_t ldX,
            const de_param_args_t *pargs, void *out, int64_t ld_out, uint8_t *ok);

int de_eval_sum_certificate(de_ctx_t *ctx, de_program_t *prog, const void *X, int64_t N, int64_t ldX,
                            const de_param_args_t *pargs, uint8_t *ok, uint8_t *certified, double *max_abs);

int de_eval_grad(de_ctx_t *ctx, de_program_t *prog, const void *X, int64_t N, int64_t ldX,
                 const de_param_args_t *pargs, int mode, void *out, int64_t ld_out, void *grad,
                 const int64_t *grad_offsets, uint8_t *ok);

int de_eval_diff(de_ctx_t *ctx, de_program_t *prog, const void *X, int64_t N, int64_t ldX,
                 int32_t direction, void *out, void *dout, int64_t ld_out, uint8_t *ok);

typedef enum de_loss_kind {
    DE_LOSS_L2 = 0,
    DE_LOSS_L1 = 1,
    DE_LOSS_PULLBACK = 2,
    DE_LOSS_HUBER = 16,
    DE_LOSS_LOGCOSH = 17,
    DE_LOSS_L1_EPS = 18,
    DE_LOSS_L2_EPS = 19,
    DE_LOSS_QUANTILE = 20,
    DE_LOSS_LP = 21,
    DE_LOSS_LOGIT_DIST = 22,
    DE_LOSS_LOGIT_MARGIN = 23,
    DE_LOSS_L1_HINGE = 24
} de_loss_kind_t;
typedef struct de_loss_spec {
    int32_t kind;
    int32_t reserved;
    double param;
// ... 175 lines not shown
```

Baseline: 15640 billion.

## Add a tight second assured tier selected per tile from input range facts

Adds a second 'assured' instruction-stream variant that is proven under tighter input bounds (|x| <= 8, |x| >= 2^-19). Each tile tracks the min and max input magnitude while loading and picks the tight, wide or plain stream. Under the tight bounds, more validity checks can be elided when the tile's data fits. The cost is an extra stream copy, more host-side proof work, and a second ballot per tile.

After: 15850 billion, median of 6. +1.4%, better.

```diff
diff --git a/dynamicexpressions.jl_amd/api.py b/dynamicexpressions.jl_amd/api.py
--- a/dynamicexpressions.jl_amd/api.py
+++ b/dynamicexpressions.jl_amd/api.py
@@ -40,6 +40,7 @@
     "de_tape_params_to_consts", "de_eval_tree_params", "de_eval_loss_tree_params", "de_eval_loss_grad_tree_params",
     "de_tree_params_accumulate_host",
     "de_fit_tree_params_bfgs", "de_tree_params_pack_host", "de_tree_params_unpack_host",
+    "de_lower_tape_assured_fact",
 ]
 
 
@@ -521,6 +522,9 @@
     if hasattr(lib, "de_lower_tape_assured_parts"):
         lib.de_lower_tape_assured_parts.restype = i64
         lib.de_lower_tape_assured_parts.argtypes = [vp, i64, vp, i64, i32, u32, C.c_double, u32, vp, i64]
+    if hasattr(lib, "de_lower_tape_assured_fact"):
+        lib.de_lower_tape_assured_fact.restype = i64
+        lib.de_lower_tape_assured_fact.argtypes = [vp, i64, vp, i64, i32, u32, C.c_double, C.c_double, u32, vp, i64]
     lib.de_lower_tape_grad.restype = i64
     lib.de_lower_tape_grad.argtypes = [C.c_int, vp, i64, vp, i64, i32, i32, u32, C.c_int, C.c_int, vp, i64, vp]
     lib.de_eval.argtypes = [vp, vp, vp, i64, i64, C.POINTER(ParamArgs), vp, i64, vp]
@@ -822,14 +826,17 @@
     return w[:int(n)].reshape(-1, 4)
 
 
-def lower_tape_assured(tape, consts, n_features: int, xmax: float = 64.0, options: int = 7, parts: Optional[int] = None) -> np.ndarray:
+def lower_tape_assured(tape, consts, n_features: int, xmax: float = 64.0, options: int = 7, parts: Optional[int] = None,
+                       amin: Optional[float] = None) -> np.ndarray:
     lib = library()
     tape = np.ascontiguousarray(tape)
     consts = np.ascontiguousarray(consts, dtype=np.float32)
     cp = consts.ctypes.data if consts.size else None
     args = (tape.ctypes.data, len(tape), cp, consts.size, n_features, options, float(xmax))
     fn = lib.de_lower_tape_assured
-    if parts is not None:
+    if amin is not None:
+        fn, args = lib.de_lower_tape_assured_fact, args + (float(amin), 7 if parts is None else int(parts))
+    elif parts is not None:
         fn, args = lib.de_lower_tape_assured_parts, args + (int(parts),)
     n = fn(*args, None, 0)
     if n < 0:
@@ -1074,10 +1081,12 @@
         return w[:int(got)].reshape(-1, 4)
 
     def meta(self, tree: int) -> dict:
-        w = np.zeros(7, dtype=np.uint32)
-        library().de_program_dump(self._h, tree, w.ctypes.data, 7, 1)
+        w = np.zeros(8, dtype=np.uint32)
+        got = library().de_program_dump(self._h, tree, w.ctypes.data, 8, 1)
+        if got < 8:
+            w[7] = w[5]
         return dict(n_slots=int(w[0]), host_ok_eval=bool(w[1]), host_ok_grad=bool(w[2]), uses_params=bool(w[3]), waves=int(w[4]),
-                    assured=bool(w[5]), assured_valid=bool(w[6]))
+                    assured=bool(w[5]), assured_valid=bool(w[6]), assured_tiers=int(w[7]))
 
     def dump_stage(self, tree: int, which: int) -> np.ndarray:
         lib = library()
diff --git a/dynamicexpressions.jl_amd/csrc/de_api_eval.cpp b/dynamicexpressions.jl_amd/csrc/de_api_eval.cpp
--- a/dynamicexpressions.jl_amd/csrc/de_api_eval.cpp
+++ b/dynamicexpressions.jl_amd/csrc/de_api_eval.cpp
@@ -312,8 +312,10 @@
     a.waves = p->waves;
     a.wave_slots = p->n_slots;
     a.var_stride = p->var_stride;
-    a.assured = p->assured && p->assured_valid && p->var_stride != 0;
+    a.assured = p->assured && p->assured_valid && p->var_stride != 0 ? p->assured_tiers : 0;
     a.assured_xmax = (float)p->assured_xmax;
+    a.assured_tight_xmax = (float)p->assured_tight_xmax;
+    a.assured_tight_amin = (float)p->assured_tight_amin;
     if (cr) {
         a.code = p->d_cert_code;
         a.code_off = p->d_cert_off;
diff --git a/dynamicexpressions.jl_amd/csrc/de_api_internal.h b/dynamicexpressions.jl_amd/csrc/de_api_internal.h
--- a/dynamicexpressions.jl_amd/csrc/de_api_internal.h
+++ b/dynamicexpressions.jl_amd/csrc/de_api_internal.h
@@ -147,6 +147,9 @@
     double assured_xmax = 64.0;
     uint32_t assured_parts = 0;
     std::vector<uint32_t> aids;
+    int assured_tiers_cfg = 2, assured_tiers = 0, assured_tiers_room = 0;
+    double assured_tight_xmax = 8.0, assured_tight_amin = 0x1p-19;
+    std::vector<uint32_t> aids2;
     uint64_t end_handler = 0;
     uint64_t endv_handler[TOPX_ENDV_COUNT] = {0};
     bool threaded = false;
diff --git a/dynamicexpressions.jl_amd/csrc/de_api_program.cpp b/dynamicexpressions.jl_amd/csrc/de_api_program.cpp
--- a/dynamicexpressions.jl_amd/csrc/de_api_program.cpp
+++ b/dynamicexpressions.jl_amd/csrc/de_api_program.cpp
@@ -157,23 +157,43 @@
     const int v = ap && *ap ? atoi(ap) : (int)ASSURED_PARTS_SHIPPED;
     return (uint32_t)v & ASSURED_PARTS_ALL;
 }
+static void assured_tight_env(double xmax, double *txmax, double *tamin) {
+    const char *ax = getenv("DE_ASSURED_TIGHT_XMAX"), *am = getenv("DE_ASSURED_TIGHT_AMIN");
+    double tx = ax && *ax ? (double)(float)atof(ax) : ASSURED_TIGHT_XMAX, ta = am && *am ? (double)(float)atof(am) : ASSURED_TIGHT_AMIN;
+    if (!(tx >= 0x1p-40 && tx <= 0x1p100)) tx = ASSURED_TIGHT_XMAX;
+    if (!(ta >= 0x1p-39 && ta <= 0x1p100)) ta = ASSURED_TIGHT_AMIN;
+    tx = std::min(tx, xmax);
+    *txmax = tx;
+    *tamin = std::min(ta, tx);
+}
+static int assured_tiers_env() {
+    const char *at = getenv("DE_ASSURED_TIERS");
+    return at && *at == '1' ? 1 : 2;
+}
 static int make_threaded(de_ctx *c, de_program *p, const Reuse *ru = nullptr) {
     p->threaded = false;
     p->waves = 1;
     p->var_stride = 0;
     p->ccode_w.clear();
     p->assured = p->assured_valid = false;
+    p->assured_tiers = 0;
     p->aids.clear();
+    p->aids2.clear();
     if (p->assured_cfg == 0) {
         if (ru && ru->old && ru->old->assured_cfg != 0) {
             p->assured_cfg = ru->old->assured_cfg;
             p->assured_xmax = ru->old->assured_xmax;
             p->assured_parts = ru->old->assured_parts;
+            p->assured_tiers_cfg = ru->old->assured_tiers_cfg;
+            p->assured_tight_xmax = ru->old->assured_tight_xmax;
+            p->assured_tight_amin = ru->old->assured_tight_amin;
         } else {
             const char *as = getenv("DE_ASSURED");
             p->assured_parts = assured_parts_env();
             p->assured_cfg = ((as && *as == '0') || p->assured_parts == 0) ? -1 : 1;
             p->assured_xmax = assured_xmax_env();
+            p->assured_tiers_cfg = assured_tiers_env();
+            assured_tight_env(p->assured_xmax, &p->assured_tight_xmax, &p->assured_tight_amin);
         }
     }
     dbg_lap(nullptr);
@@ -380,8 +400,13 @@
         else { r.lo = lo; r.hi = hi; }
     }
 }
-static void assured_link_trees(de_program *p, const uint64_t *table, int64_t tb, int64_t te, bool touched_only = false) {
-    BoundInstr *cw = p->ccode_w.data();
+static void assure_program_tree(const de_program *p, int tier, int32_t i0, int32_t i1, AssuredInstr *info) {
+    if (tier == 2) assure_tree_fact(p->fbcode.data() + i0, (size_t)(i1 - i0), p->n_features, p->assured_tight_xmax, p->assured_tight_amin, info, p->assured_parts);
+    else assure_tree(p->fbcode.data() + i0, (size_t)(i1 - i0), p->n_features, p->assured_xmax, info, p->assured_parts);
+}
+static void assured_link_trees(de_program *p, const uint64_t *table, int64_t tb, int64_t te, bool touched_only = false, int tier = 1) {
+    BoundInstr *cw = p->ccode_w.data() + (size_t)(tier - 1) * p->ccode.size();
+    std::vector<uint32_t> &aids = tier == 2 ? p->aids2 : p->aids;
     std::vector<AssuredInstr> info;
     auto name_next = [](BoundInstr &r, uint64_t handler) { r.lo = (uint32_t)handler; r.hi = (uint32_t)(handler >> 32); };
     auto ev_of = [&](int64_t t) -> int {
@@ -393,12 +418,12 @@
         if (i1 <= i0) continue;
         if (touched_only && p->const_off[(size_t)t + 1] == p->const_off[(size_t)t]) continue;
         info.resize((size_t)(i1 - i0));
-        assure_tree(p->fbcode.data() + i0, (size_t)(i1 - i0), p->n_features, p->assured_xmax, info.data(), p->assured_parts);
+        assure_program_tree(p, tier, i0, i1, info.data());
         const size_t h = (size_t)p->ccode_off[(size_t)t];
         const int ev = ev_of(t);
         for (int32_t i = i0; i < i1; i++) {
             const uint32_t id = info[(size_t)(i - i0)].id;
-            p->aids[(size_t)i] = id;
+            aids[(size_t)i] = id;
             const uint64_t handler = (i == i1 - 1 && ev >= 0) ? (topx_enda_of(id) >= 0 && id != p->fbcode[(size_t)i].bop ? table[TOPX_ENDA_BASE + (uint32_t)topx_enda_of(id)] : p->endv_handler[ev])
                                      : id == p->fbcode[(size_t)i].bop ? p->handler_base + p->tcode[(size_t)i].bop : table[id];
             if (i > i0) name_next(cw[h + (size_t)(i - i0) - 1], handler);
@@ -410,9 +435,21 @@
     }
 }
 static void make_assured(de_program *p, const uint64_t *table) {
+    const bool tight = p->assured_tiers_room ? p->assured_tiers_room >= 2
+                                             : p->assured_tiers_cfg >= 2 && (p->assured_tight_xmax < p->assured_xmax || p->assured_tight_amin > assured_wide_amin(p->assured_parts));
     p->ccode_w = p->ccode;
+    if (tight) p->ccode_w.insert(p->ccode_w.end(), p->ccode.begin(), p->ccode.end());
     p->aids.assign(p->fbcode.size(), 0u);
-    parallel_tree_ranges(p->n_trees, [&](int, int64_t tb, int64_t te) { assured_link_trees(p, table, tb, te); });
+    p->aids2.assign(tight ? p->fbcode.size() : 0, 0u);
+    parallel_tree_ranges(p->n_trees, [&](int, int64_t tb, int64_t te) {
+        assured_link_trees(p, table, tb, te);
+        if (tight) assured_link_trees(p, table, tb, te, false, 2);
+    });
+    if (tight && !p->assured_tiers_room && p->aids2 == p->aids) {
+        p->ccode_w.resize(p->ccode.size());
+        p->aids2.clear();
+    }
+    p->assured_tiers = p->aids2.empty() ? 1 : 2;
     p->var_stride = (int64_t)(p->bcode.size() + (size_t)p->n_trees + 2);
     p->assured = p->assured_valid = true;
 }
@@ -1083,7 +1120,8 @@
     }
     const size_t cbytes = (p->bcode.size() + (size_t)p->n_trees + 2) * sizeof(BoundInstr);
     {
-        const size_t nvar = p->threaded && p->var_stride ? (p->assured ? 2 : (size_t)p->waves) : 1;
+        const size_t nvar = p->threaded && p->var_stride ? (p->assured ? 1 + (size_t)p->assured_tiers : (size_t)p->waves) : 1;
+        if (p->assured) p->assured_tiers_room = p->assured_tiers;
         if (nvar > 1 && (size_t)p->var_stride * sizeof(BoundInstr) != cbytes) return fail(ctx, DE_ERR_HIP, "wave-group stream variants: stride and arena disagree");
         const size_t abytes = p->threaded ? 2 * nvar * cbytes : cbytes;
         auto al = [](size_t x) { return (x + 255) & ~(size_t)255; };
@@ -1256,7 +1294,10 @@
             uint64_t table[TOPX_TABLE];
             const hipError_t hs = eval_handler_table(p->dtype, (p->options & DE_OPT_TURBO) != 0, table);
             if (hs != hipSuccess) return fail(ctx, DE_ERR_HIP, "handler table: %s", hipGetErrorString(hs));
-            parallel_tree_ranges(p->n_trees, [&](int, int64_t tb, int64_t te) { assured_link_trees(p, table, tb, te, true); });
+            parallel_tree_ranges(p->n_trees, [&](int, int64_t tb, int64_t te) {
+                assured_link_trees(p, table, tb, te, true);
+                if (p->assured_tiers >= 2) assured_link_trees(p, table, tb, te, true, 2);
+            });
             p->assured_valid = true;
         }
         const auto t4 = now();
@@ -1821,30 +1862,37 @@
             }
         }
         if (p->assured) {
-            if (p->waves != 1 || !f32 || p->ccode_w.size() != p->ccode.size() || p->aids.size() != p->fbcode.size() || (size_t)p->var_stride < p->ccode.size())
+            const size_t tiers = (size_t)p->assured_tiers;
+            if (p->waves != 1 || !f32 || tiers < 1 || tiers > 2 || p->ccode_w.size() != tiers * p->ccode.size() || p->aids.size() != p->fbcode.size() ||
+                p->aids2.size() != (tiers == 2 ? p->fbcode.size() : 0) || (size_t)p->var_stride < p->ccode.size())
                 return bad("assured stream layout", -1, p->waves, p->ccode_w.size());
-            const BoundInstr *cw = p->ccode_w.data();
-            std::vector<AssuredInstr> info;
-            auto named = [](const BoundInstr &q) { return ((uint64_t)q.hi << 32) | q.lo; };
-            for (size_t r = 0; r < p->ccode.size(); r++)
-                if (cw[r].bop != p->ccode[r].bop || cw[r].arg != p->ccode[r].arg) return bad("assured stream: operand words differ", -1, (int64_t)r, cw[r].bop);
-            for (int64_t t = 0; t < p->n_trees; t++) {
-                const int32_t i0 = p->tcode_off[(size_t)t], i1 = p->tcode_off[(size_t)t + 1], h = p->ccode_off[(size_t)t];
-                if (i1 <= i0) continue;
-                info.resize((size_t)(i1 - i0));
-                assure_tree(p->fbcode.data() + i0, (size_t)(i1 - i0), p->n_features, p->assured_xmax, info.data(), p->assured_parts);
-                const int ev = i1 - i0 >= 2 ? topx_endv_of(p->fbcode[(size_t)i1 - 1].bop) : -1;
-                for (int32_t i = i0; i < i1; i++) {
-                    const uint32_t id = info[(size_t)(i - i0)].id;
-                    if (p->assured_valid && id != p->aids[(size_t)i]) return bad("assured stream: stale twin id", t, i - i0, p->aids[(size_t)i]);
-                    const uint32_t have = p->aids[(size_t)i];
-                    if (have >= TOPX_COUNT) return bad("assured stream: handler id", t, i - i0, have);
-                    const uint64_t want = (i == i1 - 1 && ev >= 0) ? (topx_enda_of(have) >= 0 && have != p->fbcode[(size_t)i].bop ? table[TOPX_ENDA_BASE + (uint32_t)topx_enda_of(have)] : p->endv_handler[ev])
-                                          : (have == p->fbcode[(size_t)i].bop ? p->handler_base + p->tcode[(size_t)i].bop : table[have]);
-                    if (named(cw[(size_t)(h + (i - i0) - 1)]) != want) return bad("assured stream: handler word", t, i - i0, named(cw[(size_t)(h + (i - i0) - 1)]));
+            for (size_t tier = 1; tier <= tiers; tier++) {
+                const BoundInstr *cw = p->ccode_w.data() + (tier - 1) * p->ccode.size();
+                const std::vector<uint32_t> &aids = tier == 2 ? p->aids2 : p->aids;
+                std::vector<AssuredInstr> info;
+                auto named = [](const BoundInstr &q) { return ((uint64_t)q.hi << 32) | q.lo; };
+                for (size_t r = 0; r < p->ccode.size(); r++)
+                    if (cw[r].bop != p->ccode[r].bop || cw[r].arg != p->ccode[r].arg) return bad("assured stream: operand words differ", -1, (int64_t)r, cw[r].bop);
+                for (int64_t t = 0; t < p->n_trees; t++) {
+                    const int32_t i0 = p->tcode_off[(size_t)t], i1 = p->tcode_off[(size_t)t + 1], h = p->ccode_off[(size_t)t];
+                    if (i1 <= i0) continue;
+                    info.resize((size_t)(i1 - i0));
+                    assure_program_tree(p, (int)tier, i0, i1, info.data());
+                    const int ev = i1 - i0 >= 2 ? topx_endv_of(p->fbcode[(size_t)i1 - 1].bop) : -1;
+                    for (int32_t i = i0; i < i1; i++) {
+                        const uint32_t id = info[(size_t)(i - i0)].id;
+                        if (p->assured_valid && id != aids[(size_t)i]) return bad("assured stream: stale twin id", t, i - i0, aids[(size_t)i]);
+                        const uint32_t have = aids[(size_t)i];
+                        if (have >= TOPX_COUNT) return bad("assured stream: handler id", t, i - i0, have);
+                        if (tier == 2 && have != p->aids[(size_t)i] && p->aids[(size_t)i] != p->fbcode[(size_t)i].bop && have == p->fbcode[(size_t)i].bop)
+                            return bad("assured stream: the tight tier tests what the wide tier elides", t, i - i0, have);
+                        const uint64_t want = (i == i1 - 1 && ev >= 0) ? (topx_enda_of(have) >= 0 && have != p->fbcode[(size_t)i].bop ? table[TOPX_ENDA_BASE + (uint32_t)topx_enda_of(have)] : p->endv_handler[ev])
+                                              : (have == p->fbcode[(size_t)i].bop ? p->handler_base + p->tcode[(size_t)i].bop : table[have]);
+                        if (named(cw[(size_t)(h + (i - i0) - 1)]) != want) return bad("assured stream: handler word", t, i - i0, named(cw[(size_t)(h + (i - i0) - 1)]));
+                    }
+                    if (ev < 0 && named(cw[(size_t)(h + (i1 - i0) - 1)]) != p->end_handler) return bad("assured stream: tree does not end in the end record", t, i1 - i0, 0);
+                    if (ev >= 0 && named(cw[(size_t)(h + (i1 - i0) - 1)]) != named(cw[(size_t)(h + (i1 - i0))])) return bad("assured stream: end-fused instruction and end record disagree", t, i1 - i0, 0);
                 }
-                if (ev < 0 && named(cw[(size_t)(h + (i1 - i0) - 1)]) != p->end_handler) return bad("assured stream: tree does not end in the end record", t, i1 - i0, 0);
-                if (ev >= 0 && named(cw[(size_t)(h + (i1 - i0) - 1)]) != named(cw[(size_t)(h + (i1 - i0))])) return bad("assured stream: end-fused instruction and end record disagree", t, i1 - i0, 0);
             }
         }
     }
@@ -1866,15 +1914,18 @@
         if (cap < 7) return 5;
         words[5] = p->threaded && p->assured ? 1u : 0u;
         words[6] = p->threaded && assured_valid ? 1u : 0u;
-        return 7;
-    }
-    if (which == 4) {
-        if (!p->threaded || !p->assured) return 0;
+        if (cap < 8) return 7;
+        words[7] = p->threaded && p->assured ? (uint32_t)p->assured_tiers : 0u;
+        return 8;
+    }
+    if (which == 4 || which == 5) {
+        if (!p->threaded || !p->assured || (which == 5 && p->assured_tiers < 2)) return 0;
+        const std::vector<uint32_t> &aids = which == 5 ? p->aids2 : p->aids;
         const int32_t b0 = p->tcode_off[(size_t)tree], b1 = p->tcode_off[(size_t)tree + 1];
         const int64_t nb = (int64_t)(b1 - b0) * 4;
         if (!words || cap < nb) return nb;
         std::memcpy(words, p->fbcode.data() + b0, (size_t)nb * 4);
-        for (int32_t i = b0; i < b1; i++) words[(size_t)(i - b0) * 4] = p->aids[(size_t)i];
+        for (int32_t i = b0; i < b1; i++) words[(size_t)(i - b0) * 4] = aids[(size_t)i];
         return nb;
     }
     if (which == 2) {
@@ -1984,8 +2035,13 @@
 }
 int64_t de_lower_tape_assured_parts(const de_tape_node_t *nodes, int64_t n_nodes, const void *consts, int64_t n_consts, int32_t n_features,
                                     uint32_t options, double xmax, uint32_t parts, double *out, int64_t cap) {
+    return de_lower_tape_assured_fact(nodes, n_nodes, consts, n_consts, n_features, options, xmax, assured_wide_amin(parts), parts, out, cap);
+}
+int64_t de_lower_tape_assured_fact(const de_tape_node_t *nodes, int64_t n_nodes, const void *consts, int64_t n_consts, int32_t n_features,
+                                   uint32_t options, double xmax, double amin, uint32_t parts, double *out, int64_t cap) {
     if (parts & ~ASSURED_PARTS_ALL) return -DE_ERR_INVALID_ARG;
     if (!(xmax >= 0x1p-40 && xmax <= 0x1p100)) return -DE_ERR_INVALID_ARG;
+    if (!(amin >= 0x1p-40 && amin <= xmax)) return -DE_ERR_INVALID_ARG;
     int64_t nw = lower_tape_stage_impl(DE_F32, nodes, n_nodes, consts, n_consts, n_features, 0, options, 3, nullptr, 0);
     if (nw < 0) return nw;
     try {
@@ -1995,7 +2051,7 @@
         const int64_t n = (int64_t)f.size() * 6;
         if (!out || cap < n) return n;
         std::vector<AssuredInstr> info(f.size());
-        assure_tree(f.data(), f.size(), n_features, xmax, info.data(), parts);
+        assure_tree_fact(f.data(), f.size(), n_features, xmax, amin, info.data(), parts);
         for (size_t i = 0; i < f.size(); i++) {
             double *o = out + 6 * i;
             o[0] = info[i].acc.lo; o[1] = info[i].acc.hi; o[2] = info[i].acc.amin; o[3] = info[i].acc.fin ? 1.0 : 0.0;
diff --git a/dynamicexpressions.jl_amd/csrc/de_bind.cpp b/dynamicexpressions.jl_amd/csrc/de_bind.cpp
--- a/dynamicexpressions.jl_amd/csrc/de_bind.cpp
+++ b/dynamicexpressions.jl_amd/csrc/de_bind.cpp
@@ -281,9 +281,13 @@
 }
 
 void assure_tree(const BoundInstr *f, size_t n, int n_features, double xmax, AssuredInstr *out, uint32_t parts) {
+    assure_tree_fact(f, n, n_features, xmax, assured_wide_amin(parts), out, parts);
+}
+
+void assure_tree_fact(const BoundInstr *f, size_t n, int n_features, double xmax, double amin, AssuredInstr *out, uint32_t parts) {
     static thread_local std::vector<AssuredVal> slots;
     slots.clear();
-    const AssuredVal feature{-xmax, xmax, (parts & ASSURED_PART_FUSED_DIV) ? 0x1p-39 : 0x1p-40, true};
+    const AssuredVal feature{-xmax, xmax, amin, true};
     auto row_val = [&](uint32_t row) -> AssuredVal {
         if (row < (uint32_t)n_features) return feature;
         const size_t s = row - (uint32_t)n_features;
diff --git a/dynamicexpressions.jl_amd/csrc/de_bind.h b/dynamicexpressions.jl_amd/csrc/de_bind.h
--- a/dynamicexpressions.jl_amd/csrc/de_bind.h
+++ b/dynamicexpressions.jl_amd/csrc/de_bind.h
@@ -211,6 +211,9 @@
     uint32_t bits;
 };
 void assure_tree(const BoundInstr *f, size_t n, int n_features, double xmax, AssuredInstr *out, uint32_t parts);
+constexpr double assured_wide_amin(uint32_t parts) { return (parts & 8u ) ? 0x1p-39 : 0x1p-40; }
+constexpr double ASSURED_TIGHT_XMAX = 8.0, ASSURED_TIGHT_AMIN = 0x1p-19;
+void assure_tree_fact(const BoundInstr *f, size_t n, int n_features, double xmax, double amin, AssuredInstr *out, uint32_t parts);
 
 void bind_tree(const Instr *code, size_t n, bool early_exit, int n_features, std::vector<BoundInstr> *out, int param_row_base = -1, int slot_shift = 0);
 
diff --git a/dynamicexpressions.jl_amd/csrc/de_kernels.h b/dynamicexpressions.jl_amd/csrc/de_kernels.h
--- a/dynamicexpressions.jl_amd/csrc/de_kernels.h
+++ b/dynamicexpressions.jl_amd/csrc/de_kernels.h
@@ -70,8 +70,8 @@
     bool *compacted;
     int32_t waves, wave_slots;
     int64_t var_stride;
-    bool assured = false;
-    float assured_xmax = 0.0f;
+    int32_t assured = 0;
+    float assured_xmax = 0.0f, assured_tight_xmax = 0.0f, assured_tight_amin = 0.0f;
     void *cert_max;
 };
 constexpr int DE_PRIO_MAX_F = 8;
diff --git a/dynamicexpressions.jl_amd/csrc/de_kernels.hip b/dynamicexpressions.jl_amd/csrc/de_kernels.hip
--- a/dynamicexpressions.jl_amd/csrc/de_kernels.hip
+++ b/dynamicexpressions.jl_amd/csrc/de_kernels.hip
@@ -50,10 +50,18 @@
     T loss_param;
     const double *fit_ystats;
     int32_t assured;
-    float assured_xmax;
+    float assured_xmax, assured_tight_xmax, assured_tight_amin;
 };
-__device__ __forceinline__ bool assured_value_ok(float v, float xmax) { return (__builtin_fabsf(v) <= xmax) & (__builtin_fabsf(v) >= 0x1p-39f); }
-__device__ __forceinline__ bool assured_value_ok(double, float) { return false; }
+struct TileFact {
+    uint32_t hi = 0u, lo = 0xFFFFFFFFu;
+    __device__ __forceinline__ void see(float v) {
+        const uint32_t m = __float_as_uint(v) & 0x7FFFFFFFu;
+        hi = hi > m ? hi : m;
+        lo = lo < m ? lo : m;
+    }
+    __device__ __forceinline__ void see(double) {}
+    __device__ __forceinline__ bool holds(float xmax, float amin) const { return ((int)(hi <= __float_as_uint(xmax)) & (int)(lo >= __float_as_uint(amin))) != 0; }
+};
 
 
 __device__ __forceinline__ TileMap map_block_grouped(uint32_t bid, int32_t n_chunks, int64_t n_tiles, uint32_t grp) {
@@ -1284,7 +1292,7 @@
     int32_t co_first = 0;
     if (a.skip_flagged && tA + (tid & 63) < tB) co_first = a.code_off[tA + (tid & 63)];
     constexpr bool ASSURABLE = WW == 1 && !PARAMS && sizeof(T) == 4 && DE_TBLK == 64;
-    bool x_ok = true;
+    TileFact x_fact;
     {
         const uint32_t F = (uint32_t)a.F;
         const uint32_t total = (uint32_t)TILE * F;
@@ -1321,7 +1329,7 @@
                         uint32_t j = a.f_magic ? __umulhi(e, a.f_magic) : e;
                         uint32_t f = e - j * F;
                         DE_UNROLL for (int c = 0; c < VW; c++) {
-                            if constexpr (ASSURABLE) x_ok &= assured_value_ok(buf[u][c], a.assured_xmax);
+                            if constexpr (ASSURABLE) x_fact.see(buf[u][c]);
                             rows[f * (ROWV * VW) + j] = buf[u][c];
                             ++f;
                             if (f == F) { f = 0; ++j; }
@@ -1334,7 +1342,7 @@
             for (uint32_t e = stid; e < total; e += SBLK) {
                 const uint32_t j = e / F, f = e - j * F;
                 const T v = src[e];
-                if constexpr (ASSURABLE) x_ok &= assured_value_ok(v, a.assured_xmax);
+                if constexpr (ASSURABLE) x_fact.see(v);
                 rows[f * (ROWV * VW) + j] = v;
             }
         } else {
@@ -1343,7 +1351,7 @@
                 int64_t jj = base + j;
                 jj = jj < last ? jj : last;
                 const T v = a.X[f + a.ldX * jj];
-                if constexpr (ASSURABLE) x_ok &= assured_value_ok(v, a.assured_xmax);
+                if constexpr (ASSURABLE) x_fact.see(v);
                 rows[f * (ROWV * VW) + j] = v;
             }
         }
@@ -1383,8 +1391,15 @@
     }
     __syncthreads();
 
-    const bool assured_tile = ASSURABLE && a.assured != 0 && __ballot(!x_ok) == 0ull;
-    const ConstU4Ptr code = (ConstU4Ptr)(uintptr_t)(a.code + (WW > 1 ? (int64_t)wave * a.var_stride : (assured_tile ? a.var_stride : (int64_t)0)));
+    int assured_var = 0;
+    if constexpr (ASSURABLE) {
+        if (a.assured != 0) {
+            const bool wide = __ballot(!x_fact.holds(a.assured_xmax, 0x1p-39f)) == 0ull;
+            const bool tight = a.assured > 1 && __ballot(!x_fact.holds(a.assured_tight_xmax, a.assured_tight_amin)) == 0ull;
+            assured_var = wide ? (tight ? 2 : 1) : 0;
+        }
+    }
+    const ConstU4Ptr code = (ConstU4Ptr)(uintptr_t)(a.code + (WW > 1 ? (int64_t)wave * a.var_stride : (int64_t)assured_var * a.var_stride));
     const uint32_t list_at = (WW > 1 && wave > 0) ? a.list_off + (uint32_t)(wave - 1) * DE_SKIPLIST_BYTES : 0u;
     const ConstI32Ptr code_off = (ConstI32Ptr)(uintptr_t)a.code_off;
     const bool full = base + TILE <= a.N;
@@ -1852,10 +1867,12 @@
     if (env_int("DE_DEBUG_NO_STORE", 0)) a.vec_store = 2;
     const int WW = (TBLK == 64 && (e.waves == 2 || e.waves == 4 || e.waves == 8) && (!e.uses_params || e.n_prows > 0)) ? e.waves : 1;
     a.var_stride = WW > 1 ? e.var_stride : 0;
-    a.assured = (WW == 1 && TBLK == 64 && sizeof(T) == 4 && e.assured && e.var_stride != 0 && !e.uses_params) ? 1 : 0;
+    a.assured = (WW == 1 && TBLK == 64 && sizeof(T) == 4 && e.assured && e.var_stride != 0 && !e.uses_params) ? (e.assured >= 2 ? 2 : 1) : 0;
     a.assured_xmax = e.assured_xmax;
+    a.assured_tight_xmax = e.assured_tight_xmax;
+    a.assured_tight_amin = e.assured_tight_amin;
     if (a.assured) a.var_stride = e.var_stride;
-    const unsigned n_variants = a.var_stride ? (a.assured ? 2u : (unsigned)WW) : 1u;
+    const unsigned n_variants = a.var_stride ? (a.assured ? 1u + (unsigned)a.assured : (unsigned)WW) : 1u;
     int32_t tpc, nch, nc0;
     plan_chunks(e.n_trees, a.n_tiles, &nch, &tpc, &nc0, WW);
     a.trees_per_chunk = tpc;
diff --git a/include/de_hip.h b/include/de_hip.h
--- a/include/de_hip.h
+++ b/include/de_hip.h
@@ -111,6 +111,8 @@
                               int32_t n_features, uint32_t options, double xmax, double *out, int64_t cap);
 int64_t de_lower_tape_assured_parts(const de_tape_node_t *nodes, int64_t n_nodes, const void *consts, int64_t n_consts,
                                     int32_t n_features, uint32_t options, double xmax, uint32_t parts, double *out, int64_t cap);
+int64_t de_lower_tape_assured_fact(const de_tape_node_t *nodes, int64_t n_nodes, const void *consts, int64_t n_consts,
+                                   int32_t n_features, uint32_t options, double xmax, double amin, uint32_t parts, double *out, int64_t cap);
 int64_t de_lower_tape_complex(int dtype, const de_tape_node_t *nodes, int64_t n_nodes, const void *consts,
                               int64_t n_consts, int32_t n_features, int32_t n_params, uint32_t options,
                               uint32_t *words, int64_t cap, int32_t *meta);
```
